# zju3dv/OnePose_Plus_Plus

Measured on NVIDIA H100. Metric: query images/sec (512x512, 5k 3D pts), higher is better.
Workload: dtype fp16 hi+lo operand pairs, 3 wgmma MMAs per K-step, fp32 accumulate (fp32-grade)

## Files before the change

### onepose_plus_plus_b200/csrc/opp_gemm.cu

```cuda
#include <cstdarg>
#include <cstdio>
#include <cstdlib>
#include <cstring>
#include <mutex>

#include "../../include/opp_b200.h"
#include "opp_gemm.cuh"

namespace opp {

static thread_local char g_last_error[512] = "";
void set_last_error(const char* fmt, ...) {
  va_list ap;
  va_start(ap, fmt);
  vsnprintf(g_last_error, sizeof(g_last_error), fmt, ap);
  va_end(ap);
}
const char* last_error() { return g_last_error; }

typedef CUresult (*EncodeTiledFn)(CUtensorMap*, CUtensorMapDataType, cuuint32_t, void*,
                                  const cuuint64_t*, const cuuint64_t*, const cuuint32_t*,
                                  const cuuint32_t*, CUtensorMapInterleave, CUtensorMapSwizzle,
                                  CUtensorMapL2promotion, CUtensorMapFloatOOBfill);

static EncodeTiledFn get_encode_fn() {
  static EncodeTiledFn fn = nullptr;
  static std::once_flag once;
  std::call_once(once, [] {
    void* p = nullptr;
    cudaDriverEntryPointQueryResult q;
    if (cudaGetDriverEntryPoint("cuTensorMapEncodeTiled", &p, cudaEnableDefault, &q) ==
            cudaSuccess &&
        q == cudaDriverEntryPointSuccess)
      fn = reinterpret_cast<EncodeTiledFn>(p);
  });
  return fn;
}

int num_sms() {
  static int n = 0;
  if (n == 0) {
    int dev = 0;
    if (cudaGetDevice(&dev) != cudaSuccess) return 132;
    if (cudaDeviceGetAttribute(&n, cudaDevAttrMultiProcessorCount, dev) != cudaSuccess) n = 132;
  }
  return n;
}

static int make_map(CUtensorMap* map, const void* ptr, int rank, const uint64_t* dims,
                    const uint64_t* strides_elems, const uint32_t* box) {
  EncodeTiledFn fn = get_encode_fn();
  if (!fn) {
    set_last_error("cuTensorMapEncodeTiled entry point unavailable (no CUDA driver?)");
    return OPP_ERR_CUDA;
  }
  OPP_REQUIRE((reinterpret_cast<uintptr_t>(ptr) & 15) == 0, "TMA base pointer not 16B aligned");
  OPP_REQUIRE(box[0] == 64 || box[0] == 32, "TMA inner box %u is not one swizzle row", box[0]);
  cuuint64_t gdim[5], gstr[4];
  cuuint32_t bdim[5], estr[5];
  for (int i = 0; i < rank; ++i) {
    gdim[i] = dims[i];
    bdim[i] = box[i];
    estr[i] = 1;
    OPP_REQUIRE(box[i] >= 1 && box[i] <= 256, "TMA box dim %d = %u out of range", i, box[i]);
  }
  for (int i = 0; i + 1 < rank; ++i) {
    gstr[i] = strides_elems[i] * 2;
    OPP_REQUIRE((gstr[i] & 15) == 0, "TMA stride %d (%llu B) not a multiple of 16", i,
                (unsigned long long)gstr[i]);
  }
  CUresult r = fn(map, CU_TENSOR_MAP_DATA_TYPE_FLOAT16, rank, const_cast<void*>(ptr), gdim, gstr,
                  bdim, estr, CU_TENSOR_MAP_INTERLEAVE_NONE,
                  box[0] == 32 ? CU_TENSOR_MAP_SWIZZLE_64B : CU_TENSOR_MAP_SWIZZLE_128B,
                  CU_TENSOR_MAP_L2_PROMOTION_L2_256B, CU_TENSOR_MAP_FLOAT_OOB_FILL_NONE);
  if (r != CUDA_SUCCESS) {
    set_last_error("cuTensorMapEncodeTiled failed with CUresult %d (rank %d dims %llu %llu %llu)",
                   (int)r, rank, (unsigned long long)dims[0], (unsigned long long)dims[1],
                   (unsigned long long)(rank > 2 ? dims[2] : 0));
    return OPP_ERR_CUDA;
  }
  return OPP_OK;
}

static int map_rows(CUtensorMap* map, const void* ptr, long long k, long long rows,
                    long long batches, long long ld, long long batch_stride, int box_rows, int bk = kBlockK) {
  uint64_t dims[3] = {(uint64_t)k, (uint64_t)rows, (uint64_t)batches};
  uint64_t str[2] = {(uint64_t)ld, (uint64_t)batch_stride};
  uint32_t box[3] = {(uint32_t)bk, (uint32_t)box_rows, 1};
  return make_map(map, ptr, 3, dims, str, box);
}

static void log_tile_once(int a_mode, const GemmShape& s, const char* epi) {
  static int on = -1;
  if (on < 0) {
    const char* e = getenv("OPP_LOG_TILES");
    on = e ? atoi(e) : 0;
  }
  if (!on) return;
  static std::mutex mu;
  static char seen[256][128];
  static int n_seen = 0;
  char key[128];
  snprintf(key, sizeof(key), "mode %d n %d block_n %d mma_n %d k %d conv_c %d stages %d alias %d cluster %d pair %d bk %d",
           a_mode, s.n_total, s.block_n, s.mma_n, s.k_chunks * kBlockK, s.conv_c, s.stages, s.acc_alias,
           s.cluster, s.pair, s.bk);
  std::lock_guard<std::mutex> lock(mu);
  if (on == 2) {
    fprintf(stderr, "opp gemm tile: %s epi %s\n", key, epi);
    return;
  }
  for (int i = 0; i < n_seen; ++i)
    if (!strcmp(seen[i], key)) return;
  if (n_seen < 256) strcpy(seen[n_seen++], key);
  fprintf(stderr, "opp gemm tile: %s\n", key);
}

template <int A_MODE, class Epi, bool DYN = false>
static int launch(const TensorMaps& maps, GemmShape s, const typename Epi::Params& ep,
                  cudaStream_t stream, const int* rows_dev = nullptr, int rows_mult = 1) {
  {
    static int dbg = -1;
    if (dbg < 0) {
      const char* e = getenv("OPP_DEBUG_SKIP");
      dbg = e ? atoi(e) : 0;
    }
    s.debug_skip = dbg;
    static int cap = -1;
    if (cap < 0) {
      const char* e = getenv("OPP_STAGES");
      cap = e ? atoi(e) : 0;
    }
    OPP_REQUIRE(s.mma_n >= EpiMinMmaN<Epi>::value, "GEMM tile width %d below the epilogue's minimum %d",
                s.mma_n, EpiMinMmaN<Epi>::value);
    OPP_REQUIRE(s.mma_n > 0 && gemm_pick_stages<Epi>(s, cap),
                "GEMM tile N=%d (split %d) does not fit in shared memory", s.block_n, s.split);
  }
  const int smem = gemm_smem_bytes<Epi>(s);
  log_tile_once(A_MODE, s, Epi::kName);
  OPP_REQUIRE(s.bk == kBlockK || (s.bk == 32 && A_MODE != A_ROWS), "ring slot width %d not compiled for mode %d",
              s.bk, A_MODE);
  const void* kern;
  if constexpr (DYN) kern = (const void*)gemm_kernel_dyn<A_MODE, Epi>;
  else kern = (const void*)gemm_kernel<A_MODE, Epi>;
  if constexpr (A_MODE != A_ROWS) {
    if (s.bk == 32) {
      if constexpr (DYN) kern = (const void*)gemm_kernel_dyn<A_MODE, Epi, 32>;
      else kern = (const void*)gemm_kernel<A_MODE, Epi, 32>;
    }
  }
  static unsigned long long attr_done[2] = {0, 0};
  unsigned long long& done = attr_done[s.bk == 32];
  int dev = 0;
  OPP_CHECK_CUDA(cudaGetDevice(&dev));
  if (dev < 64 && !((done >> dev) & 1ull)) {
    OPP_CHECK_CUDA(
        cudaFuncSetAttribute(kern, cudaFuncAttributeMaxDynamicSharedMemorySize, 227 * 1024));
    done |= 1ull << dev;
  }
  const long long total = (long long)s.batches * s.msup * s.n_tiles;
  if (total == 0) return OPP_OK;
  const int max_clusters = num_sms() / s.cluster;
  const int n_clusters = (int)(total < max_clusters ? total : max_clusters);
  cudaLaunchConfig_t cfg = {};
  cfg.gridDim = dim3(n_clusters * s.cluster);
  cfg.blockDim = dim3(gemm_threads(Epi::kGroups));
  cfg.dynamicSmemBytes = smem;
  cfg.stream = stream;
  cudaLaunchAttribute attr[2];
  attr[0].id = cudaLaunchAttributeClusterDimension;
  attr[0].val.clusterDim.x = s.cluster;
  attr[0].val.clusterDim.y = 1;
  attr[0].val.clusterDim.z = 1;
  attr[1].id = cudaLaunchAttributeProgrammaticStreamSerialization;
  attr[1].val.programmaticStreamSerializationAllowed = 1;
  cfg.attrs = attr;
  cfg.numAttrs = pdl_enabled() ? 2 : 1;
  void* kargs[5] = {(void*)&maps, (void*)&s, (void*)&ep, (void*)&rows_dev, (void*)&rows_mult};
  cudaError_t le = cudaLaunchKernelExC(&cfg, kern, kargs);
  if (le != cudaSuccess) {
    set_last_error("cudaLaunchKernelEx failed: %s (grid %d cluster %d pair %d smem %d stages %d "
                   "acc_alias %d block_n %d m_tiles %d n_tiles %d batches %d)",
                   cudaGetErrorString(le), n_clusters * s.cluster, s.cluster, s.pair, smem, s.stages,
                   s.acc_alias, s.block_n, s.m_tiles, s.n_tiles, s.batches);
    return OPP_ERR_CUDA;
  }
  return OPP_OK;
}

static int pick_cluster(int block_n, int m_tiles);

static void pick_grouping(GemmShape& s) {
  s.pair = 0;
  s.cluster = pick_cluster(s.block_n, s.m_tiles);
  s.msup = (s.m_tiles + s.cluster - 1) / s.cluster;
}

static int pick_cluster(int block_n, int m_tiles) {
  static int forced = -1;
  if (forced < 0) {
    const char* e = getenv("OPP_CLUSTER");
    forced = e ? atoi(e) : 0;
  }
  int c = forced > 1 ? forced : 2;
  while (c > 1 && (mma_width_for(block_n) % (8 * c) != 0 || m_tiles < c)) c >>= 1;
  return c;
}

static int conv_chunk_k(int ksize, int c_out_pad) {
  static int forced = -1;
  if (forced < 0) {
    const char* e = getenv("OPP_CONV_BK");
    forced = e ? atoi(e) : 0;
  }
  if (forced == 32 || forced == 64) return forced;
  return ksize == 3 && c_out_pad > 128 ? 32 : 64;
}

static int pick_block_n(int n) {
  if (n <= 256) return (n + 15) & ~15;
  if (n % 256 == 0) return 256;
  if (n % 128 == 0) return 128;
  return 256;
}

static void split_n_for_latency(GemmShape& s) {
  static int on = -1;
  if (on < 0) {
    const char* e = getenv("OPP_NSPLIT");
    on = e ? atoi(e) : 1;
  }
  if (!on) return;
  const int max_clusters = num_sms() / s.cluster;
  while (s.block_n >= 128 && s.block_n % 64 == 0 && s.n_total % (s.block_n / 2) == 0 &&
         (long long)s.batches * s.msup * s.n_tiles * 2 <= max_clusters) {
    s.block_n /= 2;
    s.n_tiles = s.n_total / s.block_n;
  }
}

static void ln_nsplit_cluster(GemmShape& s) {
  static int on = -1;
  if (on < 0) {
    const char* e = getenv("OPP_LN_NSPLIT");
    on = e ? atoi(e) : 1;
  }
  if (!on || s.n_total != 256 || s.block_n != 256) return;
  if ((long long)s.batches * s.m_tiles > num_sms() / 2) return;
  s.pair = 2;
  s.cluster = 2;
  s.msup = s.m_tiles;
  s.block_n = 128;
  s.n_tiles = 1;
}

template <class Epi>
static int fit_tile(GemmShape& s, int min_mma_n = 64) {
  for (;;) {
    s.mma_n = mma_width_for(s.block_n);
    if (s.mma_n < min_mma_n) s.mma_n = min_mma_n;
    GemmShape t = s;
    if (gemm_pick_stages<Epi>(t)) return OPP_OK;
    OPP_REQUIRE(s.pair == 0 && s.block_n > 16, "GEMM tile N=%d (split %d) does not fit in shared memory",
                s.block_n, s.split);
    s.block_n = (s.block_n / 2 + 15) & ~15;
    s.n_tiles = (s.n_total + s.block_n - 1) / s.block_n;
  }
}

static int setup_rows(TensorMaps& maps, GemmShape& s, const void* a0, int k0, const void* a1,
                      int k1, const void* w, int w_batched, int batches, long long rows, int n,
                      int split, int n_align = 16, int a0_shared = 0, int nsplit_ok = 0,
                      int min_mma_n = 64) {
  OPP_REQUIRE(a0 && w, "null operand");
  OPP_REQUIRE(k0 > 0 && k0 % 64 == 0 && k1 % 64 == 0, "K (%d,%d) must be multiples of 64", k0,
              k1);
  OPP_REQUIRE(n > 0 && n % n_align == 0, "N=%d must be a multiple of %d", n, n_align);
  OPP_REQUIRE(batches > 0 && rows > 0, "empty GEMM");
  const int planes = split ? 2 : 1;
  memset(&s, 0, sizeof(s));
  s.batches = batches;
  s.rows = (int)rows;
  s.m_tiles = (int)((rows + kBlockM - 1) / kBlockM);
  s.block_n = pick_block_n(n);
  OPP_REQUIRE(s.block_n % 16 == 0 && s.block_n <= 256, "bad block_n %d", s.block_n);
  s.n_tiles = (n + s.block_n - 1) / s.block_n;
  s.n_total = n;
  s.bk = kBlockK;
  s.k_chunks_a0 = k0 / 64;
  s.k_chunks = (k0 + k1) / 64;
  s.b_batched = w_batched;
  s.split = split ? 1 : 0;
  s.a0_lo = k0;
  s.a1_lo = k1;
  s.b_lo = k0 + k1;
  s.a0_shared = a0_shared ? 1 : 0;
  const long long ld0 = (long long)planes * k0, ld1 = (long long)planes * k1;
  int rc = map_rows(&maps.a[0], a0, ld0, rows, a0_shared ? 1 : batches, ld0, rows * ld0, kBlockM);
  if (rc) return rc;
  if (k1 > 0) {
    OPP_REQUIRE(a1, "null second A operand");
    rc = map_rows(&maps.a[1], a1, ld1, rows, batches, ld1, rows * ld1, kBlockM);
    if (rc) return rc;
  } else {
    maps.a[1] = maps.a[0];
  }
  maps.a[2] = maps.a[0];
  maps.a[3] = maps.a[0];
  pick_grouping(s);
  if (nsplit_ok == 1) split_n_for_latency(s);
  if (nsplit_ok == 2) ln_nsplit_cluster(s);
  rc = fit_tile<EpiLN>(s, min_mma_n);
  if (rc) return rc;
  const long long kt = (long long)planes * (k0 + k1);
  return map_rows(&maps.b, w, kt, n, w_batched ? batches : 1, kt, (long long)n * kt,
                  s.pair == 2 ? s.mma_n : s.mma_n / s.cluster);
}

}

using namespace opp;

extern "C" {

const char* opp_last_error(void) { return opp::last_error(); }

int opp_linear_act_f16(const void* a0, int k0, const void* a1, int k1, const void* w, void* out,
                       long long rows, int n, int act, int act_cols, int split,
                       opp_stream_t stream) {
  return opp_linear_act_f16_b(a0, k0, 0, a1, k1, w, out, 1, rows, n, act, act_cols, split, nullptr, stream);
}

int opp_linear_act_f16_b(const void* a0, int k0, int a0_shared, const void* a1, int k1, const void* w,
                         void* out, int batches, long long rows, int n, int act, int act_cols,
                         int split, const unsigned char* row_mask, opp_stream_t stream) {
  TensorMaps maps;
  GemmShape s;
  int rc = setup_rows(maps, s, a0, k0, a1, k1, w, 0, batches, rows, n, split, 16, a0_shared, 1);
  if (rc) return rc;
  OPP_REQUIRE(out, "null output");
  OPP_REQUIRE(act_cols % 32 == 0, "act_cols=%d must be a multiple of 32", act_cols);
  EpiStoreF16::Params ep{(__half*)out, (long long)n * (split ? 2 : 1), split ? n : 0, act,
                         act_cols, row_mask};
  return launch<A_ROWS, EpiStoreF16>(maps, s, ep, (cudaStream_t)stream);
}

int opp_linear_act_f16_out1(const void* a0, int k0, const void* a1, int k1, const void* w, void* out,
                            long long rows, int n, int act, int act_cols, const unsigned char* row_mask,
                            opp_stream_t stream) {
  TensorMaps maps;
  GemmShape s;
  int rc = setup_rows(maps, s, a0, k0, a1, k1, w, 0, 1, rows, n, 1, 16, 0, 1);
  if (rc) return rc;
  OPP_REQUIRE(out, "null output");
  OPP_REQUIRE(act_cols % 32 == 0, "act_cols=%d must be a multiple of 32", act_cols);
  EpiStoreF16::Params ep{(__half*)out, (long long)n, 0, act, act_cols, row_mask};
  return launch<A_ROWS, EpiStoreF16>(maps, s, ep, (cudaStream_t)stream);
}

int opp_linear_act_f16_dyn(const void* a0, int k0, const void* a1, int k1, const void* w, void* out,
                           long long cap_rows, const int* count, int rows_per_count, int n, int act,
                           int act_cols, int split, opp_stream_t stream) {
  TensorMaps maps;
  GemmShape s;
  int rc = setup_rows(maps, s, a0, k0, a1, k1, w, 0, 1, cap_rows, n, split);
  if (rc) return rc;
  OPP_REQUIRE(out && count && rows_per_count > 0, "bad dynamic-row arguments");
  OPP_REQUIRE(act_cols % 32 == 0, "act_cols=%d must be a multiple of 32", act_cols);
  EpiStoreF16::Params ep{(__half*)out, (long long)n * (split ? 2 : 1), split ? n : 0, act, act_cols, nullptr};
  return launch<A_ROWS, EpiStoreF16, true>(maps, s, ep, (cudaStream_t)stream, count, rows_per_count);
}

int opp_linear_ln_dyn(const void* a0, int k0, const void* a1, int k1, const void* w, const float* gamma,
                      const float* beta, float eps, const void* resid, void* out16, float* out32,
                      long long cap_rows, const int* count, int rows_per_count, int n, int split,
                      opp_stream_t stream) {
  TensorMaps maps;
  GemmShape s;
  OPP_REQUIRE(n == 128 || n == 256, "LayerNorm epilogue needs N in {128,256}, got %d", n);
  int rc = setup_rows(maps, s, a0, k0, a1, k1, w, 0, 1, cap_rows, n, split);
  if (rc) return rc;
  OPP_REQUIRE(s.n_tiles == 1 && s.block_n == n, "LayerNorm row of N=%d split across tiles", n);
  OPP_REQUIRE(gamma && beta && count && rows_per_count > 0, "bad dynamic-row arguments");
  OPP_REQUIRE(out16 || out32, "no output requested");
  EpiLN::Params ep{gamma, beta, eps, (const __half*)resid, 0, (__half*)out16,
                   (long long)n * (split ? 2 : 1), split ? n : 0, out32};
  return launch<A_ROWS, EpiLN, true>(maps, s, ep, (cudaStream_t)stream, count, rows_per_count);
}

int opp_linear_q_f16(const void* x, const void* wq, const float* ksum, void* out, int batches,
                     int rows, int d_model, float v_len, float eps, int split, int x_shared,
                     const unsigned char* row_mask, opp_stream_t stream) {
  TensorMaps maps;
  GemmShape s;
  OPP_REQUIRE(d_model == 256, "opp_linear_q_f16 supports d_model 256 (8 heads x 32), got %d",
              d_model);
  int rc = setup_rows(maps, s, x, d_model, nullptr, 0, wq, 0, batches, rows, d_model, split, 16, x_shared, 1);
  if (rc) return rc;
  OPP_REQUIRE(ksum && out, "null pointer");
  EpiQ::Params ep{(__half*)out, (long long)d_model * (split ? 2 : 1), split ? d_model : 0, ksum,
                  v_len, eps, row_mask};
  return launch<A_ROWS, EpiQ>(maps, s, ep, (cudaStream_t)stream);
}

int opp_linear_ln(const void* a0, int k0, const void* a1, int k1, const void* w, int w_batched,
                  const float* gamma, const float* beta, float eps, const void* resid,
                  int resid_shared, void* out16, float* out32, int batches, long long rows, int n,
                  int split, opp_stream_t stream) {
  TensorMaps maps;
  GemmShape s;
  OPP_REQUIRE(n == 128 || n == 256, "LayerNorm epilogue needs N in {128,256}, got %d", n);
  int rc = setup_rows(maps, s, a0, k0, a1, k1, w, w_batched, batches, rows, n, split, 16, 0, 2);
  if (rc) return rc;
  OPP_REQUIRE(s.n_tiles == 1 && s.block_n * (s.pair == 2 ? 2 : 1) == n,
              "LayerNorm row of N=%d split across tiles", n);
  OPP_REQUIRE(gamma && beta, "null LayerNorm parameters");
  OPP_REQUIRE(out16 || out32, "no output requested");
  EpiLN::Params ep{gamma, beta, eps, (const __half*)resid, resid_shared, (__half*)out16,
                   (long long)n * (split ? 2 : 1), split ? n : 0, out32};
  return launch<A_ROWS, EpiLN>(maps, s, ep, (cudaStream_t)stream);
}

int opp_conv2d_nhwc(const void* in, const void* w, const float* bias, const void* resid,
                    void* out, int batch, int in_h, int in_w, int c_in_pad, int c_out_pad,
                    int ksize, int stride, int act, float slope, void* tok, const float* pe,
                    const void* up, int split, opp_stream_t stream) {
  OPP_REQUIRE(in && w && bias, "null operand");
  OPP_REQUIRE(ksize == 1 || ksize == 3, "kernel size %d unsupported (1 or 3)", ksize);
  OPP_REQUIRE(stride == 1 || stride == 2, "stride %d unsupported", stride);
  OPP_REQUIRE(c_in_pad % 16 == 0 && c_out_pad % 16 == 0 && c_out_pad <= 256,
              "channel counts must be padded to multiples of 16 (got %d -> %d)", c_in_pad,
              c_out_pad);
  OPP_REQUIRE(stride == 1 || (in_h % 2 == 0 && in_w % 2 == 0), "stride 2 needs even H, W");
  OPP_REQUIRE(out || tok, "no output requested");
  const int planes = split ? 2 : 1;
  const int pad = ksize / 2;
  const int out_h = (in_h + 2 * pad - ksize) / stride + 1;
  const int out_w = (in_w + 2 * pad - ksize) / stride + 1;
  TensorMaps maps;
  GemmShape s;
  memset(&s, 0, sizeof(s));
  s.batches = batch;
  s.rows = out_h * out_w;
  s.tile_w = 16;
  s.tile_h = 8;
  s.tiles_x = (out_w + s.tile_w - 1) / s.tile_w;
  s.tiles_y = (out_h + s.tile_h - 1) / s.tile_h;
  s.m_tiles = s.tiles_x * s.tiles_y;
  s.block_n = c_out_pad;
  s.n_tiles = 1;
  s.n_total = c_out_pad;
  s.conv_c = c_in_pad;
  s.bk = conv_chunk_k(ksize, c_out_pad);
  s.conv_cchunks = (c_in_pad + 63) / 64;
  s.k_chunks = ksize * ksize * s.conv_cchunks;
  s.conv_kw = ksize;
  s.conv_pad = pad;
  s.conv_stride = stride;
  s.out_w = out_w;
  s.out_h = out_h;
  s.split = split ? 1 : 0;
  const long long C = (long long)planes * c_in_pad;
  const __half* base = (const __half*)in;
  int rc;
  if (stride == 1) {
    uint64_t dims[5] = {(uint64_t)c_in_pad, (uint64_t)planes, (uint64_t)in_w, (uint64_t)in_h, (uint64_t)batch};
    uint64_t str[4] = {(uint64_t)c_in_pad, (uint64_t)C, (uint64_t)(in_w * C), (uint64_t)((long long)in_h * in_w * C)};
    uint32_t box[5] = {(uint32_t)s.bk, 1, (uint32_t)s.tile_w, (uint32_t)s.tile_h, 1};
    rc = make_map(&maps.a[0], base, 5, dims, str, box);
    if (rc) return rc;
    maps.a[1] = maps.a[2] = maps.a[3] = maps.a[0];
  } else {
    for (int py = 0; py < 2; ++py)
      for (int px = 0; px < 2; ++px) {
        uint64_t dims[5] = {(uint64_t)c_in_pad, (uint64_t)planes, (uint64_t)(in_w / 2),
                            (uint64_t)(in_h / 2), (uint64_t)batch};
        uint64_t str[4] = {(uint64_t)c_in_pad, (uint64_t)(2 * C), (uint64_t)(2LL * in_w * C),
                           (uint64_t)((long long)in_h * in_w * C)};
        uint32_t box[5] = {(uint32_t)s.bk, 1, (uint32_t)s.tile_w, (uint32_t)s.tile_h, 1};
        rc = make_map(&maps.a[py * 2 + px], base + ((long long)py * in_w + px) * C, 5, dims, str,
                      box);
        if (rc) return rc;
      }
  }
  const long long kplane = (long long)ksize * ksize * c_in_pad;
  s.b_lo = (int)kplane;
  const long long kt = kplane * planes;
  pick_grouping(s);
  split_n_for_latency(s);
  rc = up ? fit_tile<EpiConvUp>(s) : fit_tile<EpiConv>(s);
  if (rc) return rc;
  rc = map_rows(&maps.b, w, kt, c_out_pad, 1, kt, (long long)c_out_pad * kt, s.mma_n / s.cluster, s.bk);
  if (rc) return rc;
  OPP_REQUIRE(!up || (out_h % 2 == 0 && out_w % 2 == 0 && out_h >= 4 && out_w >= 4),
              "fused upsample-add needs even output dims >= 4 (got %d x %d)", out_h, out_w);
  EpiConvParams ep{(__half*)out, (long long)c_out_pad * planes, split ? c_out_pad : 0, bias,
                     (const __half*)resid, act, slope, (__half*)tok, pe, (const __half*)up,
                     out_h / 2, out_w / 2,
                     up ? (float)(out_h / 2 - 1) / (float)(out_h - 1) : 0.f,
                     up ? (float)(out_w / 2 - 1) / (float)(out_w - 1) : 0.f};
  if (up) return launch<A_CONV, EpiConvUp>(maps, s, ep, (cudaStream_t)stream);
  return launch<A_CONV, EpiConv>(maps, s, ep, (cudaStream_t)stream);
}

int opp_conv_win_pitch(int win) {
  static int pack5 = -1;
  if (pack5 < 0) {
    const char* e = getenv("OPP_WIN5_PACK");
    pack5 = e ? atoi(e) : 0;
  }
  return (win == 5 && pack5) ? 5 : 8;
}

int opp_conv_win(const void* in, const void* w, const float* bias, void* out, const long long* b_ids,
                 const long long* j_ids, int matches, const int* count, int batch, int in_h, int in_w,
                 int c_in_pad, int c_out_pad, int win, int wc, int stride, int org, int act,
                 float slope, int split, opp_stream_t stream) {
  OPP_REQUIRE(in && w && bias && out, "null operand");
  OPP_REQUIRE(win == 5 || win == 7, "window side %d unsupported (5 or 7)", win);
  OPP_REQUIRE(c_in_pad % 16 == 0 && c_out_pad % 16 == 0 && c_out_pad <= 256,
              "channel counts must be padded to multiples of 16 (got %d -> %d)", c_in_pad, c_out_pad);
  OPP_REQUIRE(matches >= 0 && (j_ids == nullptr) == (b_ids == nullptr), "bad match list");
  OPP_REQUIRE(!j_ids || (wc > 0 && stride > 0 && batch > 0 && in_h > 0 && in_w > 0),
              "dense-input window convolution needs the map size, wc and stride");
  if (matches == 0) return OPP_OK;
  const int planes = split ? 2 : 1;
  TensorMaps maps;
  GemmShape s;
  memset(&s, 0, sizeof(s));
  s.batches = 1;
  const int pitch = opp_conv_win_pitch(win);
  s.tile_w = pitch;
  s.tile_h = win;
  s.tiles_x = 128 / (pitch * win);
  s.tiles_y = 1;
  s.rows = matches * pitch * win;
  s.m_tiles = (matches + s.tiles_x - 1) / s.tiles_x;
  s.block_n = c_out_pad;
  s.n_tiles = 1;
  s.n_total = c_out_pad;
  s.conv_c = c_in_pad;
  s.bk = conv_chunk_k(3, c_out_pad);
  OPP_REQUIRE(pitch == 8 || s.bk == 64, "OPP_WIN5_PACK needs 64-wide ring slots (layer has %d)", s.bk);
  s.conv_cchunks = (c_in_pad + 63) / 64;
  s.k_chunks = 9 * s.conv_cchunks;
  s.conv_kw = 3;
  s.conv_pad = 1;
  s.conv_stride = 1;
  s.out_w = pitch;
  s.out_h = win;
  s.split = split ? 1 : 0;
  const long long C = (long long)planes * c_in_pad;
  int rc;
  {
    const uint64_t iw = j_ids ? in_w : 8, ih = j_ids ? in_h : win + 2, ib = j_ids ? batch : matches;
    uint64_t dims[5] = {(uint64_t)c_in_pad, (uint64_t)planes, iw, ih, ib};
    uint64_t str[4] = {(uint64_t)c_in_pad, (uint64_t)C, (uint64_t)(iw * C), (uint64_t)(ih * iw * C)};
    uint32_t box[5] = {(uint32_t)s.bk, 1, (uint32_t)pitch, (uint32_t)win, 1};
    rc = make_map(&maps.a[0], in, 5, dims, str, box);
    if (rc) return rc;
    maps.a[1] = maps.a[2] = maps.a[3] = maps.a[0];
  }
  const long long kplane = 9LL * c_in_pad;
  s.b_lo = (int)kplane;
  const long long kt = kplane * planes;
  pick_grouping(s);
  rc = fit_tile<EpiWin>(s);
  if (rc) return rc;
  rc = map_rows(&maps.b, w, kt, c_out_pad, 1, kt, (long long)c_out_pad * kt, s.mma_n / s.cluster, s.bk);
  if (rc) return rc;
  EpiWin::Params ep{(__half*)out, (long long)c_out_pad * planes, split ? c_out_pad : 0, bias, act, slope,
                    b_ids, j_ids, wc, stride, org, in_h, in_w};
  if (count) return launch<A_WIN, EpiWin, true>(maps, s, ep, (cudaStream_t)stream, count, pitch * win);
  return launch<A_WIN, EpiWin>(maps, s, ep, (cudaStream_t)stream);
}

int opp_sim_lse(const void* a, const void* b, float* part_m, float* part_s, int batches, int rows,
                int cols, int k, float scale, int split, opp_stream_t stream) {
  TensorMaps maps;
  GemmShape s;
  int rc = setup_rows(maps, s, a, k, nullptr, 0, b, 1, batches, rows, cols, split, 1);
  if (rc) return rc;
  EpiLse::Params ep{part_m, part_s, scale};
  return launch<A_ROWS, EpiLse>(maps, s, ep, (cudaStream_t)stream);
}

int opp_sim_conf(const void* a, const void* b, const float* lse_own, const float* lse_other,
                 int own_is_pt, float* conf, float* part_val, int* part_idx, int batches,
                 int rows, int cols, int k, float scale, int split, opp_stream_t stream) {
  TensorMaps maps;
  GemmShape s;
  int rc = setup_rows(maps, s, a, k, nullptr, 0, b, 1, batches, rows, cols, split, 1);
  if (rc) return rc;
  EpiConf::Params ep{lse_own, lse_other, scale, own_is_pt, conf, part_val, part_idx};
  return launch<A_ROWS, EpiConf>(maps, s, ep, (cudaStream_t)stream);
}

int opp_sim_lse_cols_rows(const void* a, const void* b, float* part_m, float* part_s, float* col_m,
                          float* col_s, int batches, int rows, int cols, int k, float scale, int split,
                          const unsigned char* col_mask, const int* row_count, opp_stream_t stream) {
  TensorMaps maps;
  GemmShape s;
  int rc = setup_rows(maps, s, a, k, nullptr, 0, b, 1, batches, rows, cols, split, 1, 0, 0,
                      EpiLseCol::kMinMmaN);
  if (rc) return rc;
  OPP_REQUIRE(part_m && part_s && col_m && col_s, "null pointer");
  OPP_REQUIRE(!(col_mask && row_count), "col_mask and row_count are not combined");
  EpiLseColParams ep{part_m, part_s, scale, col_m, col_s, (rows + 31) / 32, col_mask};
  if (row_count) {
    EpiLseColRowsParams epr{ep, row_count};
    return launch<A_ROWS, EpiLseColRows>(maps, s, epr, (cudaStream_t)stream);
  }
  if (col_mask) return launch<A_ROWS, EpiLseColMasked>(maps, s, ep, (cudaStream_t)stream);
  return launch<A_ROWS, EpiLseCol>(maps, s, ep, (cudaStream_t)stream);
}

int opp_sim_lse_cols(const void* a, const void* b, float* part_m, float* part_s, float* col_m,
                     float* col_s, int batches, int rows, int cols, int k, float scale, int split,
                     const unsigned char* col_mask, opp_stream_t stream) {
  return opp_sim_lse_cols_rows(a, b, part_m, part_s, col_m, col_s, batches, rows, cols, k, scale, split,
                               col_mask, nullptr, stream);
}

int opp_sim_conf_colmax_rows(const void* a, const void* b, const float* lse_own, const float* lse_other,
                             float* conf, float* part_val, int* part_idx, unsigned* colmax, int batches,
                             int rows, int cols, int k, float scale, int split, const int* row_count,
                             opp_stream_t stream) {
  TensorMaps maps;
  GemmShape s;
  int rc = setup_rows(maps, s, a, k, nullptr, 0, b, 1, batches, rows, cols, split, 1, 0, 0,
                      EpiConfCol::kMinMmaN);
  if (rc) return rc;
  OPP_REQUIRE(lse_own && lse_other && part_val && part_idx && colmax, "null pointer");
  OPP_CHECK_CUDA(cudaMemsetAsync(colmax, 0, (size_t)batches * cols * sizeof(unsigned),
                                 (cudaStream_t)stream));
  EpiConfColParams ep{lse_own, lse_other, scale, conf, part_val, part_idx, colmax};
  if (row_count) {
    EpiConfColRowsParams epr{ep, row_count};
    return launch<A_ROWS, EpiConfColRows>(maps, s, epr, (cudaStream_t)stream);
  }
  return launch<A_ROWS, EpiConfCol>(maps, s, ep, (cudaStream_t)stream);
}

int opp_sim_conf_colmax(const void* a, const void* b, const float* lse_own, const float* lse_other,
                        float* conf, float* part_val, int* part_idx, unsigned* colmax, int batches,
                        int rows, int cols, int k, float scale, int split, opp_stream_t stream) {
  return opp_sim_conf_colmax_rows(a, b, lse_own, lse_other, conf, part_val, part_idx, colmax, batches, rows,
                                  cols, k, scale, split, nullptr, stream);
}

int opp_sim_tiles(int cols) {
  return (cols + pick_block_n(cols) - 1) / pick_block_n(cols);
}

}
```

### onepose_plus_plus_b200/csrc/opp_gemm.cuh

```cuda
#pragma once

#include <type_traits>

#include "opp_common.cuh"

#ifndef OPP_CONV_GROUPS
#define OPP_CONV_GROUPS 2
#endif

namespace opp {

constexpr int kBlockM = 128;
constexpr int kBlockK = 64;
__host__ __device__ constexpr int gemm_a_bytes(int bk) { return kBlockM * bk * 2; }
constexpr int kMaxStages = 8;
constexpr int kEpiParamBytes = 4096;
constexpr int kMaxEpiWarps = 8;
constexpr int gemm_threads(int groups) { return 128 + 128 * groups; }
constexpr int kProducerRegs = 40;
constexpr int kMmaRegs = 232;
static_assert(128 * kProducerRegs + 256 * kMmaRegs <= 65536, "register file of one SM");
constexpr int kMmaWidths[] = {64, 128, 208, 256};
constexpr int mma_width_for(int block_n) {
  for (int w : kMmaWidths)
    if (w >= block_n) return w;
  return 0;
}

enum AMode : int { A_ROWS = 0, A_CONV = 1, A_WIN = 2 };

struct TensorMaps {
  CUtensorMap a[4];
  CUtensorMap b;
};

struct GemmShape {
  int batches;
  int rows;
  int m_tiles;
  int n_tiles;
  int n_total;
  int block_n;
  int mma_n;
  int k_chunks;
  int bk;
  int stages;
  int b_batched;
  int cluster;
  int msup;
  int pair;
  int acc_alias;
  int debug_skip;
  int split;
  int b_lo;
  int k_chunks_a0;
  int a0_lo, a1_lo;
  int a0_shared;
  int conv_cchunks;
  int conv_c;
  int conv_kw;
  int conv_pad;
  int conv_stride;
  int tile_w, tile_h;
  int tiles_x, tiles_y;
  int out_w, out_h;
};

struct EpiCtx {
  uint32_t acc;
  int b, m_tile, n_tile;
  int q;
  int a_mode;
  int n0;
  int ncols;
  int etid;
  float* smem;
  uint8_t* wstage;
  uint32_t smem_s, wstage_s;
  int group;
  int col_first, col_step;
  long long sgrow[4];
  unsigned svalid;
  int next_b, next_m_tile;
  uint8_t* extra;
  int it;
};

__device__ __forceinline__ void epi_sync(const EpiCtx& c) { named_bar_sync(1 + c.group, 128); }

template <class E, class = void>
struct EpiWarpStage {
  static constexpr int value = 32 * 80;
};
template <class E>
struct EpiWarpStage<E, std::void_t<decltype(E::kWarpStage)>> {
  static constexpr int value = E::kWarpStage;
};
template <class E, class = void>
struct EpiExtraSmem {
  static constexpr int value = 0;
};
template <class E>
struct EpiExtraSmem<E, std::void_t<decltype(E::kExtraSmem)>> {
  static constexpr int value = E::kExtraSmem;
};
template <class E>
constexpr int epi_smem_bytes() {
  return 4096 + 8 * EpiWarpStage<E>::value + EpiExtraSmem<E>::value;
}

template <class E, class = void>
struct EpiMinMmaN {
  static constexpr int value = 64;
};
template <class E>
struct EpiMinMmaN<E, std::void_t<decltype(E::kMinMmaN)>> {
  static constexpr int value = E::kMinMmaN;
};

template <class E, class = void>
struct EpiNeedsNext : std::false_type {};
template <class E>
struct EpiNeedsNext<E, std::void_t<decltype(E::kNeedsNext)>> : std::true_type {};

template <class E, class = void>
struct EpiFromRegs : std::false_type {};
template <class E>
struct EpiFromRegs<E, std::void_t<decltype(E::kFromRegs)>> : std::true_type {};

__device__ __forceinline__ bool epi_row_at(const GemmShape& s, const EpiCtx& c, int rit,
                                           long long& grow, int& row) {
  bool ok;
  if (c.a_mode == A_ROWS) {
    row = c.m_tile * kBlockM + rit;
    ok = row < s.rows;
  } else if (c.a_mode == A_WIN) {
    const int wrows = s.tiles_x * s.tile_w * s.tile_h;
    row = c.m_tile * wrows + rit;
    ok = rit < wrows && row < s.rows;
  } else {
    const int ty = c.m_tile / s.tiles_x;
    const int tx = c.m_tile - ty * s.tiles_x;
    const int ly = rit / s.tile_w;
    const int oy = ty * s.tile_h + ly;
    const int ox = tx * s.tile_w + (rit - ly * s.tile_w);
    ok = oy < s.out_h && ox < s.out_w;
    row = oy * s.out_w + ox;
  }
  grow = (long long)c.b * s.rows + row;
  return ok;
}

constexpr int kAccPad = 4;
__host__ __device__ constexpr int gemm_acc_bytes(int mma_n) { return 128 * (mma_n + kAccPad) * 4; }

__device__ __forceinline__ void acc_ld32(uint32_t waddr, float (&v)[32]) {
#pragma unroll
  for (int i = 0; i < 8; ++i) {
    const uint4 u = lds128(waddr * 4 + 16 * i);
    v[4 * i + 0] = __uint_as_float(u.x);
    v[4 * i + 1] = __uint_as_float(u.y);
    v[4 * i + 2] = __uint_as_float(u.z);
    v[4 * i + 3] = __uint_as_float(u.w);
  }
}

constexpr int kStageRowH = 80;
constexpr int kWarpStageBytes = 32 * kStageRowH;

__device__ __forceinline__ void staged_store_h32(const GemmShape& s, const EpiCtx& c, __half* out,
                                                 long long ld, int lo_off, int gcol,
                                                 const float* v, int nvalid) {
  if (s.debug_skip & 8) return;
  const int lane = threadIdx.x & 31;
  const uint32_t st = c.wstage_s;
#pragma unroll
  for (int plane = 0; plane < 2; ++plane) {
    if (plane == 1 && lo_off == 0) break;
    const uint32_t mine = st + lane * kStageRowH;
#pragma unroll
    for (int g = 0; g < 4; ++g) {
      uint4 u;
      if (plane == 0) {
        u.x = pack_half2(v[8 * g + 0], v[8 * g + 1]);
        u.y = pack_half2(v[8 * g + 2], v[8 * g + 3]);
        u.z = pack_half2(v[8 * g + 4], v[8 * g + 5]);
        u.w = pack_half2(v[8 * g + 6], v[8 * g + 7]);
      } else {
        float l[8];
#pragma unroll
        for (int j = 0; j < 8; ++j)
          l[j] = v[8 * g + j] - __half2float(__float2half_rn(v[8 * g + j]));
        u.x = pack_half2(l[0], l[1]);
        u.y = pack_half2(l[2], l[3]);
        u.z = pack_half2(l[4], l[5]);
        u.w = pack_half2(l[6], l[7]);
      }
      sts128(mine + g * 16, u);
    }
    __syncwarp();
    const int seg = lane & 3;
#pragma unroll
    for (int i = 0; i < 4; ++i) {
      const int rr = (lane >> 2) + 8 * i;
      if (((c.svalid >> i) & 1u) && seg * 8 < nvalid)
        *reinterpret_cast<uint4*>(out + c.sgrow[i] * ld + plane * lo_off + gcol + seg * 8) =
            lds128(st + rr * kStageRowH + seg * 16);
    }
    __syncwarp();
  }
}


constexpr int kFragRowH = 80;
constexpr int kFragPlaneH = 16 * kFragRowH;
constexpr int kFragRowF = 160;

__device__ __forceinline__ void sts32u(uint32_t addr, uint32_t v) {
  asm volatile("st.shared.b32 [%0], %1;" ::"r"(addr), "r"(v) : "memory");
}
__device__ __forceinline__ uint32_t lds32u(uint32_t addr) {
  uint32_t v;
  asm volatile("ld.shared.b32 %0, [%1];" : "=r"(v) : "r"(addr) : "memory");
  return v;
}
__device__ __forceinline__ float2 lds64f(uint32_t addr) {
  float2 v;
  asm volatile("ld.shared.v2.f32 {%0, %1}, [%2];" : "=f"(v.x), "=f"(v.y) : "r"(addr) : "memory");
  return v;
}

__device__ __forceinline__ void sts64f(uint32_t addr, float a, float b) {
  asm volatile("st.shared.v2.f32 [%0], {%1, %2};" ::"r"(addr), "f"(a), "f"(b) : "memory");
}

template <int N>
__device__ __forceinline__ void frag_slice(const float (&d)[N / 2], int j, float (&v)[16], float fill = 0.f) {
#pragma unroll
  for (int k = 0; k < 16; ++k) v[k] = 16 * j + k < N / 2 ? d[16 * j + k] : fill;
}

__device__ __forceinline__ void frag_add_cols(uint32_t base_s, int col, float (&v)[16]) {
  const int c0 = 2 * (threadIdx.x & 3);
#pragma unroll
  for (int ii = 0; ii < 4; ++ii) {
    const float2 b = lds64f(base_s + 4 * ((col + 8 * ii + c0) & 255));
#pragma unroll
    for (int h = 0; h < 2; ++h) {
      v[4 * ii + 2 * h] += b.x;
      v[4 * ii + 2 * h + 1] += b.y;
    }
  }
}

__device__ __forceinline__ void frag_store_h(const GemmShape& s, const EpiCtx& c, __half* out, long long ld,
                                             int lo_off, int gcol, const float (&v)[16], int nvalid) {
  if (s.debug_skip & 8) return;
  const int lane = threadIdx.x & 31, t = lane & 3, rq = lane >> 2;
  const uint32_t st = c.wstage_s;
#pragma unroll
  for (int ii = 0; ii < 4; ++ii)
#pragma unroll
    for (int h = 0; h < 2; ++h) {
      const float a = v[4 * ii + 2 * h], b = v[4 * ii + 2 * h + 1];
      const uint32_t addr = st + (rq + 8 * h) * kFragRowH + 16 * ii + 4 * t;
      sts32u(addr, pack_half2(a, b));
      if (lo_off)
        sts32u(addr + kFragPlaneH, pack_half2(a - __half2float(__float2half_rn(a)),
                                              b - __half2float(__float2half_rn(b))));
    }
  __syncwarp();
#pragma unroll
  for (int plane = 0; plane < 2; ++plane) {
    if (plane == 1 && lo_off == 0) break;
#pragma unroll
    for (int h = 0; h < 2; ++h)
      if (((c.svalid >> h) & 1u) && t * 8 < nvalid)
        *reinterpret_cast<uint4*>(out + c.sgrow[h] * ld + plane * lo_off + gcol + t * 8) =
            lds128(st + plane * kFragPlaneH + (rq + 8 * h) * kFragRowH + 16 * t);
  }
  __syncwarp();
}

__device__ __forceinline__ void frag_store_f32(const EpiCtx& c, float* out, long long ld, int gcol,
                                               const float (&v)[16], int nvalid) {
  const int lane = threadIdx.x & 31, t = lane & 3, rq = lane >> 2;
  const uint32_t st = c.wstage_s;
#pragma unroll
  for (int ii = 0; ii < 4; ++ii)
#pragma unroll
    for (int h = 0; h < 2; ++h)
      sts64f(st + (rq + 8 * h) * kFragRowF + 4 * (8 * ii + 2 * t), v[4 * ii + 2 * h], v[4 * ii + 2 * h + 1]);
  __syncwarp();
#pragma unroll
  for (int half = 0; half < 2; ++half)
#pragma unroll
    for (int h = 0; h < 2; ++h)
      if (((c.svalid >> h) & 1u) && 16 * half + 4 * t < nvalid)
        *reinterpret_cast<uint4*>(out + c.sgrow[h] * ld + gcol + 16 * half + 4 * t) =
            lds128(st + (rq + 8 * h) * kFragRowF + 64 * half + 16 * t);
  __syncwarp();
}

__device__ __forceinline__ void frag_load_issue(const EpiCtx& c, const __half* src, long long ld, int lo_off,
                                                int gcol, int nvalid) {
  const int lane = threadIdx.x & 31, t = lane & 3, rq = lane >> 2;
#pragma unroll
  for (int h = 0; h < 2; ++h) {
    const bool in = ((c.svalid >> h) & 1u) && t * 8 < nvalid;
    const __half* row = in ? src + c.sgrow[h] * ld + gcol + t * 8 : src;
    const uint32_t dst = c.wstage_s + (rq + 8 * h) * kFragRowH + 16 * t;
    cp_async16_zfill(dst, row, in ? 16 : 0);
    if (lo_off) cp_async16_zfill(dst + kFragPlaneH, in ? row + lo_off : src, in ? 16 : 0);
  }
  cp_async_commit();
}
__device__ __forceinline__ void frag_load_add(const EpiCtx& c, int lo_off, float (&v)[16]) {
  const int lane = threadIdx.x & 31, t = lane & 3, rq = lane >> 2;
  const uint32_t st = c.wstage_s;
  cp_async_wait<0>();
  __syncwarp();
#pragma unroll
  for (int plane = 0; plane < 2; ++plane) {
    if (plane == 1 && lo_off == 0) break;
#pragma unroll
    for (int ii = 0; ii < 4; ++ii)
#pragma unroll
      for (int h = 0; h < 2; ++h) {
        const uint32_t u = lds32u(st + plane * kFragPlaneH + (rq + 8 * h) * kFragRowH + 16 * ii + 4 * t);
        const float2 f = __half22float2(*reinterpret_cast<const __half2*>(&u));
        v[4 * ii + 2 * h] += f.x;
        v[4 * ii + 2 * h + 1] += f.y;
      }
  }
  __syncwarp();
}

__device__ __forceinline__ void frag_add_f32(const EpiCtx& c, const float* src, long long ld, const int (&row)[2],
                                             int gcol, int nvalid, float (&v)[16]) {
  const int lane = threadIdx.x & 31, t = lane & 3, rq = lane >> 2;
  const uint32_t st = c.wstage_s;
#pragma unroll
  for (int h = 0; h < 2; ++h)
#pragma unroll
    for (int k = 0; k < 2; ++k) {
      const int seg = t + 4 * k;
      if (((c.svalid >> h) & 1u) && seg * 4 < nvalid)
        sts128(st + (rq + 8 * h) * kFragRowF + 16 * seg,
               *reinterpret_cast<const uint4*>(src + (long long)row[h] * ld + gcol + seg * 4));
    }
  __syncwarp();
#pragma unroll
  for (int h = 0; h < 2; ++h) {
    if (!((c.svalid >> h) & 1u)) continue;
#pragma unroll
    for (int ii = 0; ii < 4; ++ii)
      if (8 * ii < nvalid) {
        const float2 f = lds64f(st + (rq + 8 * h) * kFragRowF + 4 * (8 * ii + 2 * t));
        v[4 * ii + 2 * h] += f.x;
        v[4 * ii + 2 * h + 1] += f.y;
      }
  }
  __syncwarp();
}

__device__ __forceinline__ void frag_act(int act, float slope, float (&v)[16]) {
  if (act == 1) {
#pragma unroll
    for (int k = 0; k < 16; ++k) v[k] = fmaxf(v[k], 0.f);
  } else if (act == 2) {
#pragma unroll
    for (int k = 0; k < 16; ++k) v[k] = v[k] > 0.f ? v[k] : v[k] * slope;
  }
}

__device__ __forceinline__ void epi_stage_cols(const GemmShape& s, const EpiCtx& c, const float* src) {
  if (c.it > 0 && s.n_tiles == 1) return;
  epi_sync(c);
  for (int i = c.etid; i < c.ncols; i += 128) sts32f(c.smem_s + 4 * i, src[c.n0 + i]);
  epi_sync(c);
}

struct EpiConvParams {
  __half* out;
  long long ld;
  int out_lo;
  const float* bias;
  const __half* resid;
  int act;
  float slope;
  __half* tok;
  const float* pe;
  const __half* up;
  int up_h, up_w;
  float up_sy, up_sx;
};
struct EpiConv {
  static constexpr int kGroups = OPP_CONV_GROUPS;
  static constexpr const char* kName = "conv";
  static constexpr bool kFromRegs = true;
  using Params = EpiConvParams;
  __device__ static void prefetch(const Params& p, const GemmShape& s, const EpiCtx& c) {
    if (!p.resid) return;
    const int t = threadIdx.x & 3;
#pragma unroll
    for (int h = 0; h < 2; ++h) {
      if (!((c.svalid >> h) & 1u)) continue;
      const char* row = reinterpret_cast<const char*>(p.resid + c.sgrow[h] * p.ld + c.n0);
      for (int o = 128 * t; o < c.ncols * 2; o += 512) {
        asm volatile("prefetch.global.L2 [%0];" ::"l"(row + o));
        if (p.out_lo) asm volatile("prefetch.global.L2 [%0];" ::"l"(row + 2 * p.out_lo + o));
      }
    }
  }
  template <int N>
  __device__ __forceinline__ static void run_frag(const Params& p, const GemmShape& s, const EpiCtx& c, float (&d)[N / 2]) {
    const bool has_res = p.resid != nullptr;
    if (has_res) frag_load_issue(c, p.resid, p.ld, p.out_lo, c.n0, c.ncols);
    epi_stage_cols(s, c, p.bias);
    int prow[2] = {0, 0};
#pragma unroll
    for (int h = 0; h < 2; ++h) prow[h] = (int)(c.sgrow[h] - (long long)c.b * s.rows);
#pragma unroll
    for (int j = 0; j < (N + 31) / 32; ++j) {
      const int col = 32 * j;
      if (col < c.ncols) {
        const int g0 = c.n0 + col;
        const int nvalid = c.ncols - col;
        float v[16];
        frag_slice<N>(d, j, v);
        frag_add_cols(c.smem_s, col, v);
        if (has_res) frag_load_add(c, p.out_lo, v);
        frag_act(p.act, p.slope, v);
        if (p.out) frag_store_h(s, c, p.out, p.ld, p.out_lo, g0, v, nvalid);
        if (p.tok) {
          frag_add_f32(c, p.pe, s.n_total, prow, g0, nvalid, v);
          frag_store_h(s, c, p.tok, p.ld, p.out_lo, g0, v, nvalid);
        }
        if (has_res && col + 32 < c.ncols) frag_load_issue(c, p.resid, p.ld, p.out_lo, g0 + 32, nvalid - 32);
      }
    }
  }
};

struct EpiWin {
  static constexpr int kGroups = OPP_CONV_GROUPS;
  static constexpr const char* kName = "conv_win";
  static constexpr bool kFromRegs = true;
  struct Params {
    __half* out;
    long long ld;
    int out_lo;
    const float* bias;
    int act;
    float slope;
    const long long* b_ids;
    const long long* j_ids;
    int wc;
    int stride;
    int org;
    int in_h, in_w;
  };
  __device__ static void prefetch(const Params&, const GemmShape&, const EpiCtx&) {}
  template <int N>
  __device__ __forceinline__ static void run_frag(const Params& p, const GemmShape& s, const EpiCtx& c, float (&d)[N / 2]) {
    epi_stage_cols(s, c, p.bias);
    bool inside[2] = {true, true};
#pragma unroll
    for (int h = 0; h < 2; ++h) {
      if (p.j_ids && ((c.svalid >> h) & 1u)) {
        const int rpm = s.tile_w * s.tile_h;
        const int m = (int)(c.sgrow[h] / rpm);
        const int local = (int)(c.sgrow[h] - (long long)m * rpm);
        const int ly = local / s.tile_w, lx = local - ly * s.tile_w;
        const int jj = (int)p.j_ids[m];
        const int cy = jj / p.wc;
        const int y = p.stride * cy + p.org + ly, x = p.stride * (jj - cy * p.wc) + p.org + lx;
        inside[h] = y >= 0 && y < p.in_h && x >= 0 && x < p.in_w;
      }
    }
#pragma unroll
    for (int j = 0; j < (N + 31) / 32; ++j) {
      const int col = 32 * j;
      if (col < c.ncols) {
        float v[16];
        frag_slice<N>(d, j, v);
        frag_add_cols(c.smem_s, col, v);
        frag_act(p.act, p.slope, v);
#pragma unroll
        for (int h = 0; h < 2; ++h)
          if (!inside[h]) {
#pragma unroll
            for (int ii = 0; ii < 4; ++ii) v[4 * ii + 2 * h] = v[4 * ii + 2 * h + 1] = 0.f;
          }
        frag_store_h(s, c, p.out, p.ld, p.out_lo, c.n0 + col, v, c.ncols - col);
      }
    }
  }
};

struct EpiConvUp {
  static constexpr int kGroups = OPP_CONV_GROUPS;
  static constexpr const char* kName = "conv_up";
  static constexpr bool kNeedsNext = true;
  static constexpr int kWarpStage = 2 * 32 * 80;
  using Params = EpiConvParams;

  struct Geo {
    int ymin, xmin;
  };
  __device__ static Geo window(const Params& p, const GemmShape& s, int m_tile, int q) {
    const int ty = m_tile / s.tiles_x;
    const int oy = min(ty * s.tile_h + (q * 32) / s.tile_w, s.out_h - 1);
    const int ox = min((m_tile - ty * s.tiles_x) * s.tile_w, s.out_w - 1);
    return Geo{(int)(p.up_sy * (float)oy), (int)(p.up_sx * (float)ox)};
  }
  __device__ static long long slot_pixel(const Params& p, int b, const Geo& g, int slot) {
    const int sy_ = slot / 10, sx_ = slot - sy_ * 10;
    return ((long long)b * p.up_h + min(g.ymin + sy_, p.up_h - 1)) * p.up_w + min(g.xmin + sx_, p.up_w - 1);
  }
  __device__ static void prefetch(const Params& p, const GemmShape& s, const EpiCtx& c) {
    if (c.next_b < 0) return;
    const int lane = threadIdx.x & 31;
    if (lane >= 30) return;
    const Geo g = window(p, s, c.next_m_tile, c.q);
    const char* px = reinterpret_cast<const char*>(p.up + slot_pixel(p, c.next_b, g, lane) * p.ld);
    const int bytes = (p.out_lo ? 2 : 1) * s.n_total * 2;
    for (int o = c.group * 128; o < bytes; o += 128 * kGroups) asm volatile("prefetch.global.L2 [%0];" ::"l"(px + o));
  }
  __device__ static void run(const Params& p, const GemmShape& s, const EpiCtx& c) {
    epi_sync(c);
    for (int i = c.etid; i < c.ncols; i += 128) sts32f(c.smem_s + 4 * i, p.bias[c.n0 + i]);
    epi_sync(c);
    const int lane = threadIdx.x & 31;
    const int seg = lane & 3;
    const Geo g = window(p, s, c.m_tile, c.q);
    float w00, w01, w10, w11;
    uint32_t a00, a01, a10, a11;
    {
      const int rit = c.q * 32 + lane;
      const int ty = c.m_tile / s.tiles_x;
      const int ly = rit / s.tile_w;
      const int oy = min(ty * s.tile_h + ly, s.out_h - 1);
      const int ox = min((c.m_tile - ty * s.tiles_x) * s.tile_w + (rit - ly * s.tile_w), s.out_w - 1);
      const float fy = p.up_sy * (float)oy, fx = p.up_sx * (float)ox;
      const int y0 = (int)fy, x0 = (int)fx;
      const int y1 = y0 + (y0 < p.up_h - 1 ? 1 : 0), x1 = x0 + (x0 < p.up_w - 1 ? 1 : 0);
      const float wy = fy - (float)y0, wx = fx - (float)x0;
      w00 = (1.f - wy) * (1.f - wx);
      w01 = (1.f - wy) * wx;
      w10 = wy * (1.f - wx);
      w11 = wy * wx;
      a00 = c.wstage_s + ((y0 - g.ymin) * 10 + (x0 - g.xmin)) * kStageRowH;
      a01 = c.wstage_s + ((y0 - g.ymin) * 10 + (x1 - g.xmin)) * kStageRowH;
      a10 = c.wstage_s + ((y1 - g.ymin) * 10 + (x0 - g.xmin)) * kStageRowH;
      a11 = c.wstage_s + ((y1 - g.ymin) * 10 + (x1 - g.xmin)) * kStageRowH;
    }
    int spix[4];
#pragma unroll
    for (int i = 0; i < 4; ++i) spix[i] = (int)slot_pixel(p, c.b, g, min((lane >> 2) + 8 * i, 29));
    const __half* upb = p.up + seg * 8 + c.n0;
    const bool two = p.out_lo != 0;
    uint4 nb[8];
    auto issue = [&](int col) {
      const bool ok = seg * 8 < c.ncols - col;
#pragma unroll
      for (int i = 0; i < 4; ++i) {
        const __half* px = upb + (long long)spix[i] * p.ld + col;
        nb[i] = ok ? *reinterpret_cast<const uint4*>(px) : make_uint4(0, 0, 0, 0);
        nb[4 + i] = (ok && two) ? *reinterpret_cast<const uint4*>(px + p.out_lo) : make_uint4(0, 0, 0, 0);
      }
    };
    constexpr uint32_t kLo = 32 * kStageRowH;
    auto stage = [&]() {
#pragma unroll
      for (int i = 0; i < 4; ++i) {
        const uint32_t a = c.wstage_s + ((lane >> 2) + 8 * i) * kStageRowH + seg * 16;
        sts128(a, nb[i]);
        if (two) sts128(a + kLo, nb[4 + i]);
      }
      __syncwarp();
    };
    auto blend = [&](float* v) {
#pragma unroll
      for (int q4 = 0; q4 < 4; ++q4) {
#pragma unroll
        for (int plane = 0; plane < 2; ++plane) {
          if (plane == 1 && !two) break;
          const uint32_t o = plane * kLo + q4 * 16;
          const uint4 q00 = lds128(a00 + o), q01 = lds128(a01 + o);
          const uint4 q10 = lds128(a10 + o), q11 = lds128(a11 + o);
          const __half2* h00 = reinterpret_cast<const __half2*>(&q00);
          const __half2* h01 = reinterpret_cast<const __half2*>(&q01);
          const __half2* h10 = reinterpret_cast<const __half2*>(&q10);
          const __half2* h11 = reinterpret_cast<const __half2*>(&q11);
#pragma unroll
          for (int j = 0; j < 4; ++j) {
            const float2 fa = __half22float2(h00[j]), fb = __half22float2(h01[j]);
            const float2 fc = __half22float2(h10[j]), fd = __half22float2(h11[j]);
            v[8 * q4 + 2 * j] += (w00 * fa.x + w01 * fb.x) + (w10 * fc.x + w11 * fd.x);
            v[8 * q4 + 2 * j + 1] += (w00 * fa.y + w01 * fb.y) + (w10 * fc.y + w11 * fd.y);
          }
        }
      }
      __syncwarp();
    };
    if (c.col_first < c.ncols) issue(c.col_first);
    for (int col = c.col_first; col < c.ncols; col += c.col_step) {
      float v[32];
      acc_ld32(c.acc + col, v);
#pragma unroll
      for (int q4 = 0; q4 < 8; ++q4) {
        const uint4 bq = lds128(c.smem_s + 4 * ((col + 4 * q4) & 255));
        v[4 * q4 + 0] += __uint_as_float(bq.x);
        v[4 * q4 + 1] += __uint_as_float(bq.y);
        v[4 * q4 + 2] += __uint_as_float(bq.z);
        v[4 * q4 + 3] += __uint_as_float(bq.w);
      }
      stage();
      const int ncol = col + c.col_step;
      if (ncol < c.ncols) issue(ncol);
      blend(v);
      if (p.act == 1) {
#pragma unroll
        for (int j = 0; j < 32; ++j) v[j] = fmaxf(v[j], 0.f);
      } else if (p.act == 2) {
#pragma unroll
        for (int j = 0; j < 32; ++j) v[j] = v[j] > 0.f ? v[j] : v[j] * p.slope;
      }
      staged_store_h32(s, c, p.out, p.ld, p.out_lo, c.n0 + col, v, c.ncols - col);
    }
  }
};

__device__ __forceinline__ float quad_sum(float x) {
  x += __shfl_xor_sync(0xffffffffu, x, 1);
  return x + __shfl_xor_sync(0xffffffffu, x, 2);
}
__device__ __forceinline__ float quad_max(float x) {
  x = fmaxf(x, __shfl_xor_sync(0xffffffffu, x, 1));
  return fmaxf(x, __shfl_xor_sync(0xffffffffu, x, 2));
}
__device__ __forceinline__ void quad_argmax(float& v, int& idx) {
#pragma unroll
  for (int o = 1; o <= 2; o <<= 1) {
    const float ov = __shfl_xor_sync(0xffffffffu, v, o);
    const int oi = __shfl_xor_sync(0xffffffffu, idx, o);
    if (ov > v || (ov == v && oi < idx)) {
      v = ov;
      idx = oi;
    }
  }
}

template <class Op>
__device__ __forceinline__ void col_allreduce8(float (&x)[8], Op op) {
#pragma unroll
  for (int o = 4; o <= 16; o <<= 1)
#pragma unroll
    for (int k = 0; k < 8; ++k) x[k] = op(x[k], __shfl_xor_sync(0xffffffffu, x[k], o));
}
template <class Op>
__device__ __forceinline__ float col_reduce8(float (&x)[8], Op op) {
  const int lane = threadIdx.x & 31;
#pragma unroll
  for (int lvl = 2; lvl >= 0; --lvl) {
    const int half = 1 << lvl;
    const bool up = (lane >> (2 + lvl)) & 1;
#pragma unroll
    for (int k = 0; k < half; ++k) {
      const float keep = up ? x[half + k] : x[k];
      const float send = up ? x[k] : x[half + k];
      x[k] = op(keep, __shfl_xor_sync(0xffffffffu, send, 4 << lvl));
    }
  }
  return x[0];
}
__device__ __forceinline__ int frag_lane_col() {
  const int lane = threadIdx.x & 31, rq = lane >> 2;
  return 8 * (rq >> 1) + 2 * (lane & 3) + (rq & 1);
}
__device__ __forceinline__ float pick8(const float (&x)[8], int k) {
  float r = x[0];
#pragma unroll
  for (int i = 1; i < 8; ++i) r = k == i ? x[i] : r;
  return r;
}
__device__ __forceinline__ void pair_sync(const EpiCtx& c) { named_bar_sync(5 + 2 * c.group + (c.q >> 1), 64); }

__device__ __forceinline__ void epi_stage_cols_b(const GemmShape& s, const EpiCtx& c, const float* src) {
  epi_sync(c);
  for (int i = c.etid; i < c.ncols; i += 128) sts32f(c.smem_s + 4 * i, src[(long long)c.b * s.n_total + c.n0 + i]);
  epi_sync(c);
}

struct EpiStoreF16 {
  static constexpr int kGroups = 2;
  static constexpr const char* kName = "store_f16";
  static constexpr bool kFromRegs = true;
  struct Params {
    __half* out;
    long long ld;
    int out_lo;
    int act;
    int act_cols;
    const unsigned char* row_mask;
  };
  __device__ static void prefetch(const Params&, const GemmShape&, const EpiCtx&) {}
  template <int N>
  __device__ __forceinline__ static void run_frag(const Params& p, const GemmShape& s, const EpiCtx& c, float (&d)[N / 2]) {
    bool masked[2] = {false, false};
#pragma unroll
    for (int h = 0; h < 2; ++h) masked[h] = p.row_mask && ((c.svalid >> h) & 1u) && p.row_mask[c.sgrow[h]] == 0;
#pragma unroll
    for (int j = 0; j < (N + 31) / 32; ++j) {
      const int col = 32 * j;
      if (col < c.ncols) {
        const int g0 = c.n0 + col;
        const int act = g0 < p.act_cols ? p.act : 0;
        float v[16];
        frag_slice<N>(d, j, v);
        if (act == 1) {
#pragma unroll
          for (int k = 0; k < 16; ++k) v[k] = fmaxf(v[k], 0.f);
        } else if (act == 2) {
#pragma unroll
          for (int k = 0; k < 16; ++k) v[k] = elu_plus_one_fast(v[k]);
        }
#pragma unroll
        for (int h = 0; h < 2; ++h)
          if (masked[h]) {
#pragma unroll
            for (int ii = 0; ii < 4; ++ii) v[4 * ii + 2 * h] = v[4 * ii + 2 * h + 1] = 0.f;
          }
        frag_store_h(s, c, p.out, p.ld, p.out_lo, g0, v, c.ncols - col);
      }
    }
  }
};

struct EpiQ {
  static constexpr int kGroups = 2;
  static constexpr const char* kName = "q";
  static constexpr bool kFromRegs = true;
  struct Params {
    __half* out;
    long long ld;
    int out_lo;
    const float* ksum;
    float v_len;
    float eps;
    const unsigned char* row_mask;
  };
  __device__ static void prefetch(const Params&, const GemmShape&, const EpiCtx&) {}
  template <int N>
  __device__ __forceinline__ static void run_frag(const Params& p, const GemmShape& s, const EpiCtx& c, float (&d)[N / 2]) {
    epi_stage_cols_b(s, c, p.ksum);
    const int c0 = 2 * (threadIdx.x & 3);
    bool qmasked[2] = {false, false};
#pragma unroll
    for (int h = 0; h < 2; ++h) qmasked[h] = p.row_mask && ((c.svalid >> h) & 1u) && p.row_mask[c.sgrow[h]] == 0;
#pragma unroll
    for (int j = 0; j < (N + 31) / 32; ++j) {
      const int col = 32 * j;
      if (col < c.ncols) {
        float v[16];
        frag_slice<N>(d, j, v);
        float dot[2] = {0.f, 0.f};
#pragma unroll
        for (int ii = 0; ii < 4; ++ii) {
          const float2 kk = lds64f(c.smem_s + 4 * (col + 8 * ii + c0));
#pragma unroll
          for (int h = 0; h < 2; ++h) {
            v[4 * ii + 2 * h] = elu_plus_one_fast(v[4 * ii + 2 * h]);
            v[4 * ii + 2 * h + 1] = elu_plus_one_fast(v[4 * ii + 2 * h + 1]);
            dot[h] = fmaf(v[4 * ii + 2 * h], kk.x, dot[h]);
            dot[h] = fmaf(v[4 * ii + 2 * h + 1], kk.y, dot[h]);
          }
        }
#pragma unroll
        for (int h = 0; h < 2; ++h) {
          const float qd = quad_sum(dot[h]);
          const float z = qmasked[h] ? 0.f : p.v_len / (qd + p.eps);
#pragma unroll
          for (int ii = 0; ii < 4; ++ii) {
            v[4 * ii + 2 * h] *= z;
            v[4 * ii + 2 * h + 1] *= z;
          }
        }
        frag_store_h(s, c, p.out, p.ld, p.out_lo, c.n0 + col, v, 32);
      }
    }
  }
};

struct EpiLN {
  static constexpr int kGroups = 2;
  static constexpr const char* kName = "ln";
  static constexpr bool kFromRegs = true;
  static constexpr int kExtraSmem = 2 * 128 * 8 + 64;
  static constexpr int kExchangeArrivals = 64;
  struct Params {
    const float* gamma;
    const float* beta;
    float eps;
    const __half* resid;
    int resid_shared;
    __half* out16;
    long long ld;
    int out_lo;
    float* out32;
  };
  __device__ static void prefetch(const Params& p, const GemmShape& s, const EpiCtx& c) {
    if (!p.resid) return;
    const int t = threadIdx.x & 3;
#pragma unroll
    for (int h = 0; h < 2; ++h) {
      if (!((c.svalid >> h) & 1u)) continue;
      const long long r = p.resid_shared ? c.sgrow[h] - (long long)c.b * s.rows : c.sgrow[h];
      const char* row = reinterpret_cast<const char*>(p.resid + r * p.ld + c.n0);
      for (int o = 128 * t; o < c.ncols * 2; o += 512) {
        asm volatile("prefetch.global.L2 [%0];" ::"l"(row + o));
        if (p.out_lo) asm volatile("prefetch.global.L2 [%0];" ::"l"(row + 2 * p.out_lo + o));
      }
    }
  }
  template <int N>
  __device__ __forceinline__ static void run_frag(const Params& p, const GemmShape& s, const EpiCtx& c, float (&d)[N / 2]) {
    const int lane = threadIdx.x & 31, c0 = 2 * (lane & 3);
    const __half* resid = p.resid;
    if (resid && p.resid_shared) resid -= (long long)c.b * s.rows * p.ld;
    if (resid) frag_load_issue(c, resid, p.ld, p.out_lo, c.n0, c.ncols);
    if (c.it == 0) {
      for (int i = c.etid; i < c.ncols; i += 128) {
        sts32f(c.smem_s + 4 * i, p.gamma[c.n0 + i]);
        sts32f(c.smem_s + 4 * (256 + i), p.beta[c.n0 + i]);
      }
      epi_sync(c);
    }
    float mean[2], m2[2];
#pragma unroll
    for (int h = 0; h < 2; ++h) {
      float s1 = 0.f;
#pragma unroll
      for (int i = 0; i < N / 8; ++i) s1 += d[4 * i + 2 * h] + d[4 * i + 2 * h + 1];
      mean[h] = quad_sum(s1) / (float)c.ncols;
      float s2 = 0.f;
#pragma unroll
      for (int i = 0; i < N / 8; ++i) {
        const float a = d[4 * i + 2 * h] - mean[h], b = d[4 * i + 2 * h + 1] - mean[h];
        s2 = fmaf(a, a, s2);
        s2 = fmaf(b, b, s2);
      }
      m2[h] = quad_sum(s2);
    }
    if (s.pair == 2) {
      const int par = c.it & 1;
      const int r0 = 64 * c.group + 16 * c.q + (lane >> 2);
      float2* slot = reinterpret_cast<float2*>(c.extra) + par * 128 + r0;
      uint64_t* xbar = reinterpret_cast<uint64_t*>(c.extra + 2 * 128 * 8) + par;
      const uint32_t peer = (uint32_t)(c.n_tile ^ 1);
      float2 o[2] = {make_float2(0.f, 0.f), make_float2(0.f, 0.f)};
      if ((lane & 3) == 0) {
        st_cluster_f32x2(slot, peer, mean[0], m2[0]);
        st_cluster_f32x2(slot + 8, peer, mean[1], m2[1]);
        mbar_arrive_cluster_release(xbar, peer);
        mbar_wait_cluster(xbar, (uint32_t)((c.it >> 1) & 1));
        o[0] = slot[0];
        o[1] = slot[8];
      }
#pragma unroll
      for (int h = 0; h < 2; ++h) {
        o[h].x = __shfl_sync(0xffffffffu, o[h].x, lane & ~3);
        o[h].y = __shfl_sync(0xffffffffu, o[h].y, lane & ~3);
        const float mean_a = c.n_tile == 0 ? mean[h] : o[h].x, m2a = c.n_tile == 0 ? m2[h] : o[h].y;
        const float mean_b = c.n_tile == 0 ? o[h].x : mean[h], m2b = c.n_tile == 0 ? o[h].y : m2[h];
        const float delta = mean_b - mean_a;
        mean[h] = mean_a + delta * 0.5f;
        m2[h] = m2a + m2b + delta * delta * (0.5f * (float)c.ncols);
      }
    }
    float rstd[2];
#pragma unroll
    for (int h = 0; h < 2; ++h) rstd[h] = 1.f / sqrtf(m2[h] / (float)s.n_total + p.eps);
#pragma unroll
    for (int j = 0; j < (N + 31) / 32; ++j) {
      const int col = 32 * j;
      if (col < c.ncols) {
        const int nvalid = c.ncols - col;
        float v[16];
        frag_slice<N>(d, j, v);
#pragma unroll
        for (int ii = 0; ii < 4; ++ii) {
          const float2 gq = lds64f(c.smem_s + 4 * (col + 8 * ii + c0));
          const float2 bq = lds64f(c.smem_s + 4 * (256 + col + 8 * ii + c0));
#pragma unroll
          for (int h = 0; h < 2; ++h) {
            v[4 * ii + 2 * h] = (v[4 * ii + 2 * h] - mean[h]) * rstd[h] * gq.x + bq.x;
            v[4 * ii + 2 * h + 1] = (v[4 * ii + 2 * h + 1] - mean[h]) * rstd[h] * gq.y + bq.y;
          }
        }
        if (resid) frag_load_add(c, p.out_lo, v);
        if (p.out32) frag_store_f32(c, p.out32, s.n_total, c.n0 + col, v, nvalid);
        if (p.out16) frag_store_h(s, c, p.out16, p.ld, p.out_lo, c.n0 + col, v, nvalid);
        if (resid && col + 32 < c.ncols) frag_load_issue(c, resid, p.ld, p.out_lo, c.n0 + col + 32, nvalid - 32);
      }
    }
  }
};

struct EpiLse {
  static constexpr int kGroups = 2;
  static constexpr const char* kName = "lse";
  static constexpr bool kFromRegs = true;
  struct Params {
    float* part_m;
    float* part_s;
    float scale;
  };
  __device__ static void prefetch(const Params&, const GemmShape&, const EpiCtx&) {}
  template <int N>
  __device__ __forceinline__ static void run_frag(const Params& p, const GemmShape& s, const EpiCtx& c, float (&d)[N / 2]) {
    const int c0 = 2 * (threadIdx.x & 3);
#pragma unroll
    for (int h = 0; h < 2; ++h) {
      float m = -INFINITY;
#pragma unroll
      for (int i = 0; i < N / 8; ++i)
#pragma unroll
        for (int e = 0; e < 2; ++e)
          if (8 * i + c0 + e < c.ncols) m = fmaxf(m, d[4 * i + 2 * h + e] * p.scale);
      m = quad_max(m);
      float sum = 0.f;
#pragma unroll
      for (int i = 0; i < N / 8; ++i)
#pragma unroll
        for (int e = 0; e < 2; ++e)
          if (8 * i + c0 + e < c.ncols) sum += fast_exp(d[4 * i + 2 * h + e] * p.scale - m);
      sum = quad_sum(sum);
      if ((threadIdx.x & 3) == 0 && ((c.svalid >> h) & 1u)) {
        p.part_m[c.sgrow[h] * s.n_tiles + c.n_tile] = m;
        p.part_s[c.sgrow[h] * s.n_tiles + c.n_tile] = sum;
      }
    }
  }
};

__device__ __forceinline__ void conf_store(const GemmShape& s, const EpiCtx& c, float* conf, int col,
                                           const float (&v)[16]) {
  if ((s.n_total & 3) == 0) {
    frag_store_f32(c, conf, (long long)s.n_total, c.n0 + col, v, c.ncols - col);
    return;
  }
  const int c0 = 2 * (threadIdx.x & 3);
#pragma unroll
  for (int h = 0; h < 2; ++h) {
    if (!((c.svalid >> h) & 1u)) continue;
    float* dst = conf + c.sgrow[h] * (long long)s.n_total + c.n0 + col;
#pragma unroll
    for (int ii = 0; ii < 4; ++ii)
#pragma unroll
      for (int e = 0; e < 2; ++e)
        if (col + 8 * ii + c0 + e < c.ncols) dst[8 * ii + c0 + e] = v[4 * ii + 2 * h + e];
  }
}

__device__ __forceinline__ void conf_slice(const EpiCtx& c, int col, float scale, const float (&lown)[2],
                                           bool own_is_pt, float (&v)[16], float (&best)[2], int (&bidx)[2]) {
  const int c0 = 2 * (threadIdx.x & 3);
#pragma unroll
  for (int ii = 0; ii < 4; ++ii)
#pragma unroll
    for (int e = 0; e < 2; ++e) {
      const int cl = col + 8 * ii + c0 + e;
      const float lo = lds32f(c.smem_s + 4 * (cl & 255));
#pragma unroll
      for (int h = 0; h < 2; ++h) {
        const float x2 = 2.f * (v[4 * ii + 2 * h + e] * scale);
        const float x = fast_exp(own_is_pt ? (x2 - lown[h]) - lo : (x2 - lo) - lown[h]);
        v[4 * ii + 2 * h + e] = x;
        if (cl < c.ncols && x > best[h]) {
          best[h] = x;
          bidx[h] = c.n0 + cl;
        }
      }
    }
}
__device__ __forceinline__ void conf_best_store(const GemmShape& s, const EpiCtx& c, float* part_val, int* part_idx,
                                                float (&best)[2], int (&bidx)[2]) {
#pragma unroll
  for (int h = 0; h < 2; ++h) {
    quad_argmax(best[h], bidx[h]);
    if ((threadIdx.x & 3) == 0 && ((c.svalid >> h) & 1u)) {
      part_val[c.sgrow[h] * s.n_tiles + c.n_tile] = best[h];
      part_idx[c.sgrow[h] * s.n_tiles + c.n_tile] = bidx[h];
    }
  }
}

struct EpiConf {
  static constexpr int kGroups = 2;
  static constexpr const char* kName = "conf";
  static constexpr bool kFromRegs = true;
  struct Params {
    const float* lse_own;
    const float* lse_other;
    float scale;
    int own_is_pt;
    float* conf;
    float* part_val;
    int* part_idx;
  };
  __device__ static void prefetch(const Params&, const GemmShape&, const EpiCtx&) {}
  template <int N>
  __device__ __forceinline__ static void run_frag(const Params& p, const GemmShape& s, const EpiCtx& c, float (&d)[N / 2]) {
    epi_stage_cols_b(s, c, p.lse_other);
    float lown[2], best[2] = {-1.f, -1.f};
    int bidx[2] = {c.n0, c.n0};
#pragma unroll
    for (int h = 0; h < 2; ++h) lown[h] = ((c.svalid >> h) & 1u) ? p.lse_own[c.sgrow[h]] : 0.f;
#pragma unroll
    for (int j = 0; j < (N + 31) / 32; ++j) {
      const int col = 32 * j;
      if (col < c.ncols) {
        float v[16];
        frag_slice<N>(d, j, v);
        conf_slice(c, col, p.scale, lown, p.own_is_pt != 0, v, best, bidx);
        if (p.conf) conf_store(s, c, p.conf, col, v);
      }
    }
    conf_best_store(s, c, p.part_val, p.part_idx, best, bidx);
  }
};

struct EpiLseColParams {
  float* part_m;
  float* part_s;
  float scale;
  float* col_m;
  float* col_s;
  int row_groups;
  const unsigned char* col_mask;
};
struct EpiLseColRowsParams : EpiLseColParams {
  const int* row_count;
};

__device__ __forceinline__ unsigned rows_below_count(const GemmShape& s, const EpiCtx& c, const int* row_count) {
  const long long end = (long long)c.b * s.rows + row_count[c.b];
  return c.svalid & ((c.sgrow[0] < end ? 1u : 0u) | (c.sgrow[1] < end ? 2u : 0u));
}

template <bool kMask, bool kRows = false>
struct EpiLseColT {
  static_assert(!(kMask && kRows), "query_image_mask and per-batch row counts are not combined");
  static constexpr int kGroups = 2;
  static constexpr const char* kName = kRows ? "lse_col_rows" : "lse_col";
  static constexpr bool kFromRegs = true;
  static constexpr int kMinMmaN = 128;
  using Params = std::conditional_t<kRows, EpiLseColRowsParams, EpiLseColParams>;
  __device__ static void prefetch(const Params&, const GemmShape&, const EpiCtx&) {}
  template <int N>
  __device__ __forceinline__ static void run_frag(const Params& p, const GemmShape& s, const EpiCtx& c, float (&d)[N / 2]) {
    const int lane = threadIdx.x & 31, c0 = 2 * (lane & 3);
    unsigned valid = c.svalid;
    if constexpr (kRows) valid = rows_below_count(s, c, p.row_count);
    if constexpr (kMask) {
      epi_sync(c);
      for (int i = c.etid; i < c.ncols; i += 128)
        sts32f(c.smem_s + 4 * i, p.col_mask[(long long)c.b * s.n_total + c.n0 + i] ? 0.f : -1e9f);
      epi_sync(c);
    }
#pragma unroll
    for (int i = 0; i < N / 8; ++i)
#pragma unroll
      for (int e = 0; e < 2; ++e) {
        const int cl = 8 * i + c0 + e;
        float cb_ = 0.f;
        if constexpr (kMask) cb_ = lds32f(c.smem_s + 4 * (cl & 255));
#pragma unroll
        for (int h = 0; h < 2; ++h)
          d[4 * i + 2 * h + e] = (((valid >> h) & 1u) && cl < c.ncols) ? d[4 * i + 2 * h + e] * p.scale + cb_
                                                                        : -INFINITY;
      }
#pragma unroll
    for (int h = 0; h < 2; ++h) {
      float m = -INFINITY;
#pragma unroll
      for (int i = 0; i < N / 8; ++i) m = fmaxf(m, fmaxf(d[4 * i + 2 * h], d[4 * i + 2 * h + 1]));
      m = quad_max(m);
      float sum = 0.f;
#pragma unroll
      for (int i = 0; i < N / 8; ++i)
#pragma unroll
        for (int e = 0; e < 2; ++e)
          if (8 * i + c0 + e < c.ncols) sum += fast_exp(d[4 * i + 2 * h + e] - m);
      sum = quad_sum(sum);
      if ((lane & 3) == 0 && ((valid >> h) & 1u)) {
        p.part_m[c.sgrow[h] * s.n_tiles + c.n_tile] = m;
        p.part_s[c.sgrow[h] * s.n_tiles + c.n_tile] = sum;
      }
    }
    constexpr int kSlices = (N + 31) / 32;
    float cmax[kSlices], csum[kSlices];
    const int rq = lane >> 2;
#pragma unroll
    for (int j = 0; j < kSlices; ++j) {
      cmax[j] = -INFINITY;
      csum[j] = 0.f;
      if (32 * j < c.ncols) {
        float v[16];
        frag_slice<N>(d, j, v, -INFINITY);
        float x[8];
#pragma unroll
        for (int k = 0; k < 8; ++k) x[k] = fmaxf(v[4 * (k >> 1) + (k & 1)], v[4 * (k >> 1) + 2 + (k & 1)]);
        col_allreduce8(x, [](float a, float b) { return fmaxf(a, b); });
        cmax[j] = pick8(x, rq);
#pragma unroll
        for (int k = 0; k < 8; ++k) {
          const float a = v[4 * (k >> 1) + (k & 1)], b = v[4 * (k >> 1) + 2 + (k & 1)];
          x[k] = (a == -INFINITY ? 0.f : fast_exp(a - x[k])) + (b == -INFINITY ? 0.f : fast_exp(b - x[k]));
        }
        csum[j] = col_reduce8(x, [](float a, float b) { return a + b; });
      }
    }
    const bool odd = (c.q & 1) != 0;
    const uint32_t xs = c.wstage_s + (odd ? 0 : kWarpStageBytes);
    if (odd) {
#pragma unroll
      for (int j = 0; j < kSlices; ++j) sts64f(xs + 8 * (32 * j + lane), cmax[j], csum[j]);
    }
    pair_sync(c);
    if (!odd) {
      const int rg = c.m_tile * 4 + 2 * c.group + (c.q >> 1);
      if (rg < p.row_groups) {
        const long long cbase = ((long long)c.b * p.row_groups + rg) * s.n_total + c.n0;
        const int lc = frag_lane_col();
#pragma unroll
        for (int j = 0; j < kSlices; ++j) {
          const int cl = 32 * j + lc;
          if (cl < c.ncols) {
            const float2 o = lds64f(xs + 8 * (32 * j + lane));
            const float m = fmaxf(cmax[j], o.x);
            const float sa = cmax[j] == -INFINITY ? 0.f : csum[j] * fast_exp(cmax[j] - m);
            const float sb = o.x == -INFINITY ? 0.f : o.y * fast_exp(o.x - m);
            p.col_m[cbase + cl] = m;
            p.col_s[cbase + cl] = sa + sb;
          }
        }
      }
    }
    pair_sync(c);
  }
};

using EpiLseCol = EpiLseColT<false>;
using EpiLseColMasked = EpiLseColT<true>;
using EpiLseColRows = EpiLseColT<false, true>;

struct EpiConfColParams {
  const float* lse_own;
  const float* lse_other;
  float scale;
  float* conf;
  float* part_val;
  int* part_idx;
  unsigned* colmax;
};
struct EpiConfColRowsParams : EpiConfColParams {
  const int* row_count;
};
template <bool kRows>
struct EpiConfColT {
  static constexpr int kGroups = 2;
  static constexpr const char* kName = kRows ? "conf_col_rows" : "conf_col";
  static constexpr bool kFromRegs = true;
  static constexpr int kMinMmaN = 128;
  using Params = std::conditional_t<kRows, EpiConfColRowsParams, EpiConfColParams>;
  __device__ static void prefetch(const Params&, const GemmShape&, const EpiCtx&) {}
  template <int N>
  __device__ __forceinline__ static void run_frag(const Params& p, const GemmShape& s, const EpiCtx& c, float (&d)[N / 2]) {
    const int lane = threadIdx.x & 31;
    epi_stage_cols_b(s, c, p.lse_other);
    unsigned valid = c.svalid;
    if constexpr (kRows) valid = rows_below_count(s, c, p.row_count);
    float lown[2], best[2] = {-1.f, -1.f};
    int bidx[2] = {c.n0, c.n0};
#pragma unroll
    for (int h = 0; h < 2; ++h) lown[h] = ((valid >> h) & 1u) ? p.lse_own[c.sgrow[h]] : 0.f;
    constexpr int kSlices = (N + 31) / 32;
    float cmax[kSlices];
#pragma unroll
    for (int j = 0; j < kSlices; ++j) {
      const int col = 32 * j;
      cmax[j] = 0.f;
      if (col < c.ncols) {
        float v[16];
        frag_slice<N>(d, j, v);
        conf_slice(c, col, p.scale, lown, true, v, best, bidx);
        if constexpr (kRows) {
#pragma unroll
          for (int k = 0; k < 16; ++k)
            if (!((valid >> ((k >> 1) & 1)) & 1u)) v[k] = 0.f;
        }
        if (p.conf) conf_store(s, c, p.conf, col, v);
        float x[8];
#pragma unroll
        for (int k = 0; k < 8; ++k) {
          const float a = (valid & 1u) ? v[4 * (k >> 1) + (k & 1)] : 0.f;
          const float b = (valid & 2u) ? v[4 * (k >> 1) + 2 + (k & 1)] : 0.f;
          x[k] = fmaxf(a, b);
        }
        cmax[j] = col_reduce8(x, [](float a, float b) { return fmaxf(a, b); });
      }
    }
    conf_best_store(s, c, p.part_val, p.part_idx, best, bidx);
    const bool odd = (c.q & 1) != 0;
    const uint32_t xs = c.wstage_s + (odd ? 0 : kWarpStageBytes);
    if (odd) {
#pragma unroll
      for (int j = 0; j < kSlices; ++j) sts32f(xs + 4 * (32 * j + lane), cmax[j]);
    }
    pair_sync(c);
    if (!odd) {
      unsigned* cm = p.colmax + (long long)c.b * s.n_total + c.n0;
      const int lc = frag_lane_col();
#pragma unroll
      for (int j = 0; j < kSlices; ++j) {
        const int cl = 32 * j + lc;
        const float m = fmaxf(cmax[j], lds32f(xs + 4 * (32 * j + lane)));
        if (cl < c.ncols && m > 0.f) atomicMax(cm + cl, __float_as_uint(m));
      }
    }
    pair_sync(c);
  }
};

using EpiConfCol = EpiConfColT<false>;
using EpiConfColRows = EpiConfColT<true>;

template <int R>
__device__ __forceinline__ void wgmma_fence_acc(float (&d)[R]) {
#pragma unroll
  for (int i = 0; i < R; ++i) asm volatile("" : "+f"(d[i])::"memory");
}

template <int N, int KS>
__device__ __forceinline__ void mma_k_steps(float (&d)[N / 2], bool split, uint64_t a_hi, uint64_t a_lo,
                                            uint64_t b_hi, uint64_t b_lo) {
#pragma unroll
  for (int k = 0; k < KS; ++k) wgmma_m64nNk16<N>(d, a_hi + 2 * k, b_hi + 2 * k);
  if (split) {
#pragma unroll
    for (int k = 0; k < KS; ++k) wgmma_m64nNk16<N>(d, a_hi + 2 * k, b_lo + 2 * k);
#pragma unroll
    for (int k = 0; k < KS; ++k) wgmma_m64nNk16<N>(d, a_lo + 2 * k, b_hi + 2 * k);
  }
}

template <int A_MODE, class Epi, int BK>
__device__ __forceinline__ void gemm_body(const TensorMaps& maps, const GemmShape& s,
                                          const typename Epi::Params& ep) {
  static_assert(Epi::kGroups == 2, "each of the two MMA warpgroups is one epilogue group");
  static_assert(BK == 64 || BK == 32, "K chunk of one 128B- or 64B-swizzle row");
  constexpr int kABytes = gemm_a_bytes(BK);
  extern __shared__ uint8_t smem_raw[];
  uint8_t* smem = reinterpret_cast<uint8_t*>(
      (reinterpret_cast<uintptr_t>(smem_raw) + 1023) & ~static_cast<uintptr_t>(1023));
  const int planes = s.split ? 2 : 1;
  const bool nsc = s.pair == 2;
  constexpr int kParts = kBlockK / BK;
  const int slots = s.stages * kParts;
  const int b_bytes = s.mma_n * BK * 2;
  const int a_stage = kABytes * planes;
  const int b_stage = b_bytes * planes;
  const int ring = slots * (a_stage + b_stage);
  uint8_t* smem_a = smem;
  uint8_t* smem_b = smem + slots * a_stage;
  constexpr bool kAccTile = !EpiFromRegs<Epi>::value;
  uint8_t* smem_acc = s.acc_alias ? smem : smem + ring;
  float* epi_smem = reinterpret_cast<float*>(smem + ring + (kAccTile && !s.acc_alias ? gemm_acc_bytes(s.mma_n) : 0));
  uint64_t* bars = reinterpret_cast<uint64_t*>(reinterpret_cast<uint8_t*>(epi_smem) +
                                               epi_smem_bytes<Epi>());
  uint64_t* full = bars;
  uint64_t* empty = bars + kMaxStages;
  uint64_t* accfree = bars + 2 * kMaxStages;

  constexpr int kProducerWarp = 4 * Epi::kGroups;
  const int warp = threadIdx.x >> 5;
  const int lane = threadIdx.x & 31;
  const int csize = nsc ? 1 : s.cluster;
  const int prank = s.cluster > 1 ? (int)cluster_ctarank() : 0;
  const int crank = nsc ? 0 : prank;
  const int nrank = nsc ? prank : 0;
  const uint16_t cmask = (uint16_t)((1u << csize) - 1u);
  const int cluster_id = blockIdx.x / s.cluster;
  const int n_clusters = gridDim.x / s.cluster;
  const int tiles_per_batch = s.msup * s.n_tiles;
  const int total_tiles = s.batches * tiles_per_batch;

  if (warp == kProducerWarp && lane == 0) {
    tma_prefetch_desc(&maps.a[0]);
    tma_prefetch_desc(&maps.b);
  }
  if (warp == 0 && lane == 0) {
    for (int i = 0; i < slots; ++i) {
      mbar_init(&full[i], 1);
      mbar_init(&empty[i], 2 * csize);
    }
    mbar_init(accfree, 4 * Epi::kGroups * csize);
    if constexpr (EpiExtraSmem<Epi>::value > 0) {
      uint64_t* xbar = reinterpret_cast<uint64_t*>(reinterpret_cast<uint8_t*>(epi_smem) + epi_smem_bytes<Epi>() -
                                                   EpiExtraSmem<Epi>::value + 2 * 128 * 8);
      mbar_init(&xbar[0], Epi::kExchangeArrivals);
      mbar_init(&xbar[1], Epi::kExchangeArrivals);
    }
    fence_mbar_init();
  }
  if (s.cluster > 1) cluster_sync_all(); else __syncthreads();
  pdl_sync();

  if (warp >= kProducerWarp) {
    setmaxnreg_dec<kProducerRegs>();
    if (warp == kProducerWarp) {
      int stage = 0;
      uint32_t phase = 0;
      const bool skip_b = (s.debug_skip & 1) != 0, skip_a = (s.debug_skip & 2) != 0;
      const int a_tx = A_MODE == A_WIN ? s.tiles_x * s.tile_w * s.tile_h * (BK * 2) * planes : a_stage;
      const uint32_t tx_bytes = (skip_a ? 0 : a_tx) + (skip_b ? 0 : b_stage);
      int it = 0;
      for (int t = cluster_id; t < total_tiles; t += n_clusters, ++it) {
        if (s.acc_alias && it > 0) mbar_wait(accfree, (uint32_t)((it - 1) & 1));
        const int b = t / tiles_per_batch;
        const int r = t - b * tiles_per_batch;
        const int msi = r / s.n_tiles;
        const int n_tile = nsc ? nrank : r - msi * s.n_tiles;
        const int m_tile = msi * csize + crank;
        int ox0 = 0, oy0 = 0;
        if (A_MODE == A_CONV) {
          const int ty = m_tile / s.tiles_x;
          oy0 = ty * s.tile_h;
          ox0 = (m_tile - ty * s.tiles_x) * s.tile_w;
        }
        const int bb = s.b_batched ? b : 0;
        const int nrow0 = n_tile * s.block_n;
        int win_x[5] = {0, 0, 0, 0, 0}, win_y[5] = {0, 0, 0, 0, 0}, win_z[5] = {0, 0, 0, 0, 0};
        if constexpr (A_MODE == A_WIN) {
          const int cnt = s.rows / (s.tile_w * s.tile_h);
#pragma unroll
          for (int wi = 0; wi < 5; ++wi) {
            int m = m_tile * s.tiles_x + wi;
            m = m < cnt ? m : cnt - 1;
            win_z[wi] = m;
            if (ep.j_ids) {
              const int j = (int)ep.j_ids[m];
              const int cy = j / ep.wc;
              win_z[wi] = (int)ep.b_ids[m];
              win_x[wi] = ep.stride * (j - cy * ep.wc) + ep.org - s.conv_pad;
              win_y[wi] = ep.stride * cy + ep.org - s.conv_pad;
            }
          }
        }
        int cc = 0, ky = 0, kx = 0, kb_tap = 0;
        for (int chunk = 0; chunk < s.k_chunks; ++chunk) {
          const bool first = A_MODE == A_ROWS && chunk < s.k_chunks_a0;
          const int ka = A_MODE == A_ROWS ? (first ? chunk : chunk - s.k_chunks_a0) * kBlockK : cc * kBlockK;
          const int kb = A_MODE == A_ROWS ? chunk * kBlockK : kb_tap + ka;
#pragma unroll
          for (int part = 0; part < kParts; ++part) {
            const int kp = part * BK;
            mbar_wait(&empty[stage], phase ^ 1);
            uint8_t* sa = smem_a + stage * a_stage;
            uint8_t* sb = smem_b + stage * b_stage;
            {
              if constexpr (A_MODE == A_ROWS) {
                const CUtensorMap* am = first ? &maps.a[0] : &maps.a[1];
                const int lo = first ? s.a0_lo : s.a1_lo;
                const int ba = (first && s.a0_shared) ? 0 : b;
                if (elect_one()) {
                  mbar_expect_tx(&full[stage], tx_bytes);
                  if (!skip_a) {
                    tma_load_3d(am, &full[stage], sa, ka + kp, m_tile * kBlockM, ba);
                    if (s.split) tma_load_3d(am, &full[stage], sa + kABytes, ka + kp + lo, m_tile * kBlockM, ba);
                  }
                }
              } else if constexpr (A_MODE == A_WIN) {
                const int wbytes = s.tile_w * s.tile_h * (BK * 2);
#pragma unroll
                for (int wi = 0; wi < 5; ++wi) {
                  if (wi >= s.tiles_x) break;
                  const int bx = win_x[wi] + kx, by = win_y[wi] + ky, bz = win_z[wi];
                  if (elect_one()) {
                    if (wi == 0) mbar_expect_tx(&full[stage], tx_bytes);
                    if (!skip_a) {
                      tma_load_5d(&maps.a[0], &full[stage], sa + wi * wbytes, ka + kp, 0, bx, by, bz);
                      if (s.split)
                        tma_load_5d(&maps.a[0], &full[stage], sa + kABytes + wi * wbytes, ka + kp, 1, bx, by, bz);
                    }
                  }
                }
              } else {
                int dy = ky - s.conv_pad, dx = kx - s.conv_pad, mi = 0;
                if (s.conv_stride == 2) {
                  const int py = dy & 1, px = dx & 1;
                  dy = (dy - py) >> 1;
                  dx = (dx - px) >> 1;
                  mi = py * 2 + px;
                }
                const CUtensorMap* am = &maps.a[mi];
                if (elect_one()) {
                  mbar_expect_tx(&full[stage], tx_bytes);
                  if (!skip_a) {
                    tma_load_5d(am, &full[stage], sa, ka + kp, 0, ox0 + dx, oy0 + dy, b);
                    if (s.split) tma_load_5d(am, &full[stage], sa + kABytes, ka + kp, 1, ox0 + dx, oy0 + dy, b);
                  }
                }
              }
              if (!skip_b && elect_one()) {
                if (csize == 1) {
                  tma_load_3d(&maps.b, &full[stage], sb, kb + kp, nrow0, bb);
                  if (s.split) tma_load_3d(&maps.b, &full[stage], sb + b_bytes, s.b_lo + kb + kp, nrow0, bb);
                } else {
                  const int slice = s.mma_n / csize;
                  const int soff = crank * slice * (BK * 2);
                  const int nrow = nrow0 + crank * slice;
                  tma_load_3d_mc(&maps.b, &full[stage], sb + soff, kb + kp, nrow, bb, cmask);
                  if (s.split)
                    tma_load_3d_mc(&maps.b, &full[stage], sb + b_bytes + soff, s.b_lo + kb + kp, nrow, bb, cmask);
                }
              }
            }
            __syncwarp();
            if (++stage == slots) {
              stage = 0;
              phase ^= 1;
            }
          }
          if (A_MODE != A_ROWS && ++cc == s.conv_cchunks) {
            cc = 0;
            kb_tap += s.conv_c;
            if (++kx == s.conv_kw) {
              kx = 0;
              ++ky;
            }
          }
        }
      }
    }
  } else {
    setmaxnreg_inc<kMmaRegs>();
    const int g = warp >> 2;
    const int q = warp & 3;
    EpiCtx c;
    c.etid = q * 32 + lane;
    c.q = q;
    c.a_mode = A_MODE;
    c.group = g;
    c.col_first = 32 * g;
    c.col_step = 32 * Epi::kGroups;
    c.smem = epi_smem + g * (kEpiParamBytes / 8);
    c.wstage = reinterpret_cast<uint8_t*>(epi_smem) + kEpiParamBytes + warp * EpiWarpStage<Epi>::value;
    c.extra = reinterpret_cast<uint8_t*>(epi_smem) + epi_smem_bytes<Epi>() - EpiExtraSmem<Epi>::value;
    c.smem_s = smem_u32(c.smem);
    c.wstage_s = smem_u32(c.wstage);
    const uint64_t desc_tmpl = BK == 64 ? make_kmajor_sw128_desc(0) : make_kmajor_sw64_desc(0);
    const uint32_t sa0 = ((smem_u32(smem_a) >> 4) & 0x3FFF) + g * ((64 * BK * 2) >> 4);
    const uint32_t sb0 = (smem_u32(smem_b) >> 4) & 0x3FFF;
    const uint32_t a_step = (uint32_t)a_stage >> 4, b_step = (uint32_t)b_stage >> 4;
    const uint32_t a_lo_off = kABytes >> 4, b_lo_off = (uint32_t)b_bytes >> 4;
    const bool split = s.split != 0;
    const bool is_signal = q == 0 && lane == 0;
    const uint32_t pitch = (uint32_t)(s.mma_n + kAccPad);
    const uint32_t acc_w = smem_u32(smem_acc) >> 2;
    const uint32_t r0 = 64 * g + 16 * q + (lane >> 2), c0 = 2 * (lane & 3);
    auto release = [&](int st) {
      if (is_signal) {
        if (csize == 1) mbar_arrive(&empty[st]);
        else
          for (int r = 0; r < csize; ++r) mbar_arrive_cluster(&empty[st], (uint32_t)r);
      }
    };
    int stage = 0;
    uint32_t phase = 0;
    uint32_t sa = sa0, sb = sb0;
    const int tail_steps = (A_MODE != A_ROWS && (s.conv_c & 63)) ? (s.conv_c & 63) / 16 : 4;
    int it = 0;
    for (int t = cluster_id; t < total_tiles; t += n_clusters, ++it) {
      c.b = t / tiles_per_batch;
      const int r = t - c.b * tiles_per_batch;
      const int msi = r / s.n_tiles;
      c.n_tile = nsc ? nrank : r - msi * s.n_tiles;
      c.m_tile = msi * csize + crank;
      c.n0 = c.n_tile * s.block_n;
      const int rem = s.n_total - c.n0;
      c.ncols = rem < s.block_n ? rem : s.block_n;
      if constexpr (EpiNeedsNext<Epi>::value) {
        const int tn = t + n_clusters;
        c.next_b = -1;
        c.next_m_tile = 0;
        if (tn < total_tiles) {
          c.next_b = tn / tiles_per_batch;
          c.next_m_tile = ((tn - c.next_b * tiles_per_batch) / s.n_tiles) * csize + crank;
        }
      }
      c.it = it;
      c.svalid = 0;
      if constexpr (kAccTile) {
#pragma unroll
        for (int i = 0; i < 4; ++i) {
          int rdummy;
          if (epi_row_at(s, c, q * 32 + (lane >> 2) + 8 * i, c.sgrow[i], rdummy)) c.svalid |= 1u << i;
        }
      } else {
#pragma unroll
        for (int h = 0; h < 2; ++h) {
          int rdummy;
          if (epi_row_at(s, c, (int)r0 + 8 * h, c.sgrow[h], rdummy)) c.svalid |= 1u << h;
        }
      }
      c.acc = acc_w + (uint32_t)(q * 32 + lane) * pitch;
      Epi::prefetch(ep, s, c);

      auto mma_tile = [&](auto n_c, auto tail_c) {
        constexpr int N = decltype(n_c)::value;
        constexpr int TAIL = decltype(tail_c)::value;
        float d[N / 2];
#pragma unroll
        for (int i = 0; i < N / 2; ++i) d[i] = 0.f;
        wgmma_fence_acc(d);
        int prev = -1;
        static_assert(TAIL * 16 <= BK, "a tail chunk's channels lie in its first slot");
        auto chunk_step = [&](auto ks_c, auto& acc) {
          const uint64_t a_hi = desc_tmpl | sa, b_hi = desc_tmpl | sb;
          const uint64_t a_lo = desc_tmpl | (sa + a_lo_off), b_lo = desc_tmpl | (sb + b_lo_off);
          mbar_wait_hot(&full[stage], phase);
          wgmma_fence();
          mma_k_steps<N, decltype(ks_c)::value>(acc, split, a_hi, a_lo, b_hi, b_lo);
          wgmma_commit();
          wgmma_fence_acc(acc);
          if (prev >= 0) {
            wgmma_wait<1>();
            release(prev);
          }
          prev = stage;
          sa += a_step;
          sb += b_step;
          if (++stage == slots) {
            stage = 0;
            phase ^= 1;
            sa = sa0;
            sb = sb0;
          }
        };
        auto full_chunk = [&]() {
#pragma unroll
          for (int part = 0; part < kParts; ++part) chunk_step(std::integral_constant<int, BK / 16>{}, d);
        };
        auto tail_chunk = [&]() {
          chunk_step(std::integral_constant<int, TAIL>{}, d);
          if constexpr (kParts == 2) chunk_step(std::integral_constant<int, 0>{}, d);
        };
        if constexpr (TAIL == 0) {
          for (int chunk = 0; chunk < s.k_chunks; ++chunk) full_chunk();
        } else {
          const int taps = s.k_chunks / s.conv_cchunks;
          for (int tap = 0; tap < taps; ++tap) {
            for (int cc = 1; cc < s.conv_cchunks; ++cc) full_chunk();
            tail_chunk();
          }
        }
        wgmma_wait<0>();
        wgmma_fence_acc(d);
        if (prev >= 0) release(prev);

        if constexpr (!kAccTile) {
          if (!(s.debug_skip & 4)) Epi::template run_frag<N>(ep, s, c, d);
        } else {
          named_bar_sync(4, 256);
#pragma unroll
          for (int i = 0; i < N / 8; ++i) {
            const uint32_t col = 8 * i + c0;
            sts64f((acc_w + r0 * pitch + col) * 4, d[4 * i], d[4 * i + 1]);
            sts64f((acc_w + (r0 + 8) * pitch + col) * 4, d[4 * i + 2], d[4 * i + 3]);
          }
          named_bar_sync(4, 256);
        }
      };
      auto mma_width = [&](auto tail_c) {
        switch (s.mma_n) {
          case 64:
            if constexpr (EpiMinMmaN<Epi>::value <= 64) mma_tile(std::integral_constant<int, 64>{}, tail_c);
            break;
          case 128: mma_tile(std::integral_constant<int, 128>{}, tail_c); break;
          case 208: mma_tile(std::integral_constant<int, 208>{}, tail_c); break;
          default: mma_tile(std::integral_constant<int, 256>{}, tail_c); break;
        }
      };
      if constexpr (A_MODE == A_ROWS) {
        mma_width(std::integral_constant<int, 0>{});
      } else {
        switch (tail_steps) {
          case 1: mma_width(std::integral_constant<int, 1>{}); break;
          default: mma_width(std::integral_constant<int, 0>{}); break;
        }
      }

      if constexpr (kAccTile) {
        if (!(s.debug_skip & 4)) Epi::run(ep, s, c);
        if (s.acc_alias) {
          fence_proxy_async_smem();
          __syncwarp();
          if (lane == 0) {
            if (csize == 1) mbar_arrive(accfree);
            else
              for (int r2 = 0; r2 < csize; ++r2) mbar_arrive_cluster(accfree, (uint32_t)r2);
          }
        }
      }
    }
  }

  pdl_done();
  if (s.cluster > 1) cluster_sync_all(); else __syncthreads();
}

template <int A_MODE, class Epi, int BK = kBlockK>
__global__ void __launch_bounds__(gemm_threads(Epi::kGroups), 1)
gemm_kernel(const __grid_constant__ TensorMaps maps, const GemmShape s, const typename Epi::Params ep) {
  gemm_body<A_MODE, Epi, BK>(maps, s, ep);
}

template <int A_MODE, class Epi, int BK = kBlockK>
__global__ void __launch_bounds__(gemm_threads(Epi::kGroups), 1)
gemm_kernel_dyn(const __grid_constant__ TensorMaps maps, const GemmShape s_in,
                const typename Epi::Params ep, const int* rows_dev, int rows_mult) {
  GemmShape s = s_in;
  pdl_wait();
  const int r = *rows_dev * rows_mult;
  s.rows = r < s_in.rows ? r : s_in.rows;
  const int tile_rows = A_MODE == A_WIN ? s_in.tiles_x * s_in.tile_w * s_in.tile_h : kBlockM;
  s.m_tiles = (s.rows + tile_rows - 1) / tile_rows;
  s.msup = (s.m_tiles + s_in.cluster - 1) / s_in.cluster;
  gemm_body<A_MODE, Epi, BK>(maps, s, ep);
}

inline int gemm_stage_bytes(int mma_n, int split) {
  return (gemm_a_bytes(kBlockK) + mma_n * kBlockK * 2) * (split ? 2 : 1);
}
template <class Epi>
inline int gemm_smem_bytes(const GemmShape& s) {
  const bool acc_tile = !EpiFromRegs<Epi>::value && !s.acc_alias;
  return s.stages * gemm_stage_bytes(s.mma_n, s.split) + (acc_tile ? gemm_acc_bytes(s.mma_n) : 0) +
         epi_smem_bytes<Epi>() + (2 * kMaxStages + 2) * 8 + 16 + 1024;
}
constexpr int kSmemLimit = 227 * 1024;
template <class Epi>
inline bool gemm_pick_stages(GemmShape& s, int cap = 0) {
  const int avail = kSmemLimit - epi_smem_bytes<Epi>() - 2048;
  const int sb = gemm_stage_bytes(s.mma_n, s.split);
  const int max_st = kMaxStages * s.bk / kBlockK;
  const int ab = EpiFromRegs<Epi>::value ? 0 : gemm_acc_bytes(s.mma_n);
  int st = (avail - ab) / sb;
  s.acc_alias = ab > 0 && st < 2;
  if (s.acc_alias) st = avail / sb;
  if (st > max_st) st = max_st;
  if (st > s.k_chunks * 2 && s.k_chunks * 2 >= 2) st = s.k_chunks * 2;
  if (cap > 1 && st > cap) st = cap;
  if (st < 2) st = 2;
  if (s.acc_alias && st * sb < ab) st = (ab + sb - 1) / sb;
  s.stages = st;
  return st <= max_st && gemm_smem_bytes<Epi>(s) <= kSmemLimit;
}

}
```

Before: 478.1.

## Move conv_up epilogue to register fragments and drop the smem accumulator tile

The bilinear-upsample-add epilogue (EpiConvUp) now runs directly on the wgmma accumulator fragments. Before, it first staged the whole accumulator tile into shared memory and read it back. Each warp cp.async-copies a 20-pixel upsample window into a double-buffered warp stage and blends from there, replacing the per-lane global loads. With no epilogue still using the smem accumulator tile, that tile is removed along with the acc_alias mode and its barrier, and the freed shared memory goes to more pipeline stages. The window assumes each warp's fragment rows map to one output row of at most 20 source pixels, which ties correctness to the tile geometry.

```diff
diff --git a/onepose_plus_plus_b200/csrc/opp_gemm.cu b/onepose_plus_plus_b200/csrc/opp_gemm.cu
--- a/onepose_plus_plus_b200/csrc/opp_gemm.cu
+++ b/onepose_plus_plus_b200/csrc/opp_gemm.cu
@@ -102,8 +102,8 @@
   static int n_seen = 0;
   char key[128];
   snprintf(key, sizeof(key), "mode %d n %d block_n %d mma_n %d k %d conv_c %d stages %d alias %d cluster %d pair %d bk %d",
-           a_mode, s.n_total, s.block_n, s.mma_n, s.k_chunks * kBlockK, s.conv_c, s.stages, s.acc_alias,
-           s.cluster, s.pair, s.bk);
+           a_mode, s.n_total, s.block_n, s.mma_n, s.k_chunks * kBlockK, s.conv_c, s.stages, 0, s.cluster,
+           s.pair, s.bk);
   std::lock_guard<std::mutex> lock(mu);
   if (on == 2) {
     fprintf(stderr, "opp gemm tile: %s epi %s\n", key, epi);
@@ -179,9 +179,9 @@
   cudaError_t le = cudaLaunchKernelExC(&cfg, kern, kargs);
   if (le != cudaSuccess) {
     set_last_error("cudaLaunchKernelEx failed: %s (grid %d cluster %d pair %d smem %d stages %d "
-                   "acc_alias %d block_n %d m_tiles %d n_tiles %d batches %d)",
+                   "block_n %d m_tiles %d n_tiles %d batches %d)",
                    cudaGetErrorString(le), n_clusters * s.cluster, s.cluster, s.pair, smem, s.stages,
-                   s.acc_alias, s.block_n, s.m_tiles, s.n_tiles, s.batches);
+                   s.block_n, s.m_tiles, s.n_tiles, s.batches);
     return OPP_ERR_CUDA;
   }
   return OPP_OK;
diff --git a/onepose_plus_plus_b200/csrc/opp_gemm.cuh b/onepose_plus_plus_b200/csrc/opp_gemm.cuh
--- a/onepose_plus_plus_b200/csrc/opp_gemm.cuh
+++ b/onepose_plus_plus_b200/csrc/opp_gemm.cuh
@@ -49,7 +49,6 @@
   int cluster;
   int msup;
   int pair;
-  int acc_alias;
   int debug_skip;
   int split;
   int b_lo;
@@ -67,7 +66,6 @@
 };
 
 struct EpiCtx {
-  uint32_t acc;
   int b, m_tile, n_tile;
   int q;
   int a_mode;
@@ -78,19 +76,18 @@
   uint8_t* wstage;
   uint32_t smem_s, wstage_s;
   int group;
-  int col_first, col_step;
-  long long sgrow[4];
+  long long sgrow[2];
   unsigned svalid;
-  int next_b, next_m_tile;
   uint8_t* extra;
   int it;
 };
 
 __device__ __forceinline__ void epi_sync(const EpiCtx& c) { named_bar_sync(1 + c.group, 128); }
 
+constexpr int kWarpStageBytes = 2 * 16 * 80;
 template <class E, class = void>
 struct EpiWarpStage {
-  static constexpr int value = 32 * 80;
+  static constexpr int value = kWarpStageBytes;
 };
 template <class E>
 struct EpiWarpStage<E, std::void_t<decltype(E::kWarpStage)>> {
@@ -118,15 +115,6 @@
   static constexpr int value = E::kMinMmaN;
 };
 
-template <class E, class = void>
-struct EpiNeedsNext : std::false_type {};
-template <class E>
-struct EpiNeedsNext<E, std::void_t<decltype(E::kNeedsNext)>> : std::true_type {};
-
-template <class E, class = void>
-struct EpiFromRegs : std::false_type {};
-template <class E>
-struct EpiFromRegs<E, std::void_t<decltype(E::kFromRegs)>> : std::true_type {};
 
 __device__ __forceinline__ bool epi_row_at(const GemmShape& s, const EpiCtx& c, int rit,
                                            long long& grow, int& row) {
@@ -151,69 +139,10 @@
   return ok;
 }
 
-constexpr int kAccPad = 4;
-__host__ __device__ constexpr int gemm_acc_bytes(int mma_n) { return 128 * (mma_n + kAccPad) * 4; }
-
-__device__ __forceinline__ void acc_ld32(uint32_t waddr, float (&v)[32]) {
-#pragma unroll
-  for (int i = 0; i < 8; ++i) {
-    const uint4 u = lds128(waddr * 4 + 16 * i);
-    v[4 * i + 0] = __uint_as_float(u.x);
-    v[4 * i + 1] = __uint_as_float(u.y);
-    v[4 * i + 2] = __uint_as_float(u.z);
-    v[4 * i + 3] = __uint_as_float(u.w);
-  }
-}
-
-constexpr int kStageRowH = 80;
-constexpr int kWarpStageBytes = 32 * kStageRowH;
-
-__device__ __forceinline__ void staged_store_h32(const GemmShape& s, const EpiCtx& c, __half* out,
-                                                 long long ld, int lo_off, int gcol,
-                                                 const float* v, int nvalid) {
-  if (s.debug_skip & 8) return;
-  const int lane = threadIdx.x & 31;
-  const uint32_t st = c.wstage_s;
-#pragma unroll
-  for (int plane = 0; plane < 2; ++plane) {
-    if (plane == 1 && lo_off == 0) break;
-    const uint32_t mine = st + lane * kStageRowH;
-#pragma unroll
-    for (int g = 0; g < 4; ++g) {
-      uint4 u;
-      if (plane == 0) {
-        u.x = pack_half2(v[8 * g + 0], v[8 * g + 1]);
-        u.y = pack_half2(v[8 * g + 2], v[8 * g + 3]);
-        u.z = pack_half2(v[8 * g + 4], v[8 * g + 5]);
-        u.w = pack_half2(v[8 * g + 6], v[8 * g + 7]);
-      } else {
-        float l[8];
-#pragma unroll
-        for (int j = 0; j < 8; ++j)
-          l[j] = v[8 * g + j] - __half2float(__float2half_rn(v[8 * g + j]));
-        u.x = pack_half2(l[0], l[1]);
-        u.y = pack_half2(l[2], l[3]);
-        u.z = pack_half2(l[4], l[5]);
-        u.w = pack_half2(l[6], l[7]);
-      }
-      sts128(mine + g * 16, u);
-    }
-    __syncwarp();
-    const int seg = lane & 3;
-#pragma unroll
-    for (int i = 0; i < 4; ++i) {
-      const int rr = (lane >> 2) + 8 * i;
-      if (((c.svalid >> i) & 1u) && seg * 8 < nvalid)
-        *reinterpret_cast<uint4*>(out + c.sgrow[i] * ld + plane * lo_off + gcol + seg * 8) =
-            lds128(st + rr * kStageRowH + seg * 16);
-    }
-    __syncwarp();
-  }
-}
-
 
 constexpr int kFragRowH = 80;
 constexpr int kFragPlaneH = 16 * kFragRowH;
+static_assert(kWarpStageBytes == 2 * kFragPlaneH, "the default warp stage holds both planes of a slice");
 constexpr int kFragRowF = 160;
 
 __device__ __forceinline__ void sts32u(uint32_t addr, uint32_t v) {
@@ -254,10 +183,11 @@
 }
 
 __device__ __forceinline__ void frag_store_h(const GemmShape& s, const EpiCtx& c, __half* out, long long ld,
-                                             int lo_off, int gcol, const float (&v)[16], int nvalid) {
+                                             int lo_off, int gcol, const float (&v)[16], int nvalid,
+                                             uint32_t stage_off = 0) {
   if (s.debug_skip & 8) return;
   const int lane = threadIdx.x & 31, t = lane & 3, rq = lane >> 2;
-  const uint32_t st = c.wstage_s;
+  const uint32_t st = c.wstage_s + stage_off;
 #pragma unroll
   for (int ii = 0; ii < 4; ++ii)
 #pragma unroll
@@ -398,7 +328,6 @@
 struct EpiConv {
   static constexpr int kGroups = OPP_CONV_GROUPS;
   static constexpr const char* kName = "conv";
-  static constexpr bool kFromRegs = true;
   using Params = EpiConvParams;
   __device__ static void prefetch(const Params& p, const GemmShape& s, const EpiCtx& c) {
     if (!p.resid) return;
@@ -446,7 +375,6 @@
 struct EpiWin {
   static constexpr int kGroups = OPP_CONV_GROUPS;
   static constexpr const char* kName = "conv_win";
-  static constexpr bool kFromRegs = true;
   struct Params {
     __half* out;
     long long ld;
@@ -502,133 +430,127 @@
 struct EpiConvUp {
   static constexpr int kGroups = OPP_CONV_GROUPS;
   static constexpr const char* kName = "conv_up";
-  static constexpr bool kNeedsNext = true;
-  static constexpr int kWarpStage = 2 * 32 * 80;
+  static constexpr int kWinPx = 20;
+  static constexpr int kWinBytes = 2 * kWinPx * kFragRowH;
+  static constexpr int kWarpStage = 2 * kWinBytes;
+  static_assert(kWinBytes >= kWarpStageBytes, "a window buffer also serves frag_store_h");
   using Params = EpiConvParams;
 
   struct Geo {
     int ymin, xmin;
   };
-  __device__ static Geo window(const Params& p, const GemmShape& s, int m_tile, int q) {
+  __device__ static int tile_row(const EpiCtx& c) { return 4 * c.group + c.q; }
+  __device__ static Geo window(const Params& p, const GemmShape& s, int m_tile, int row) {
     const int ty = m_tile / s.tiles_x;
-    const int oy = min(ty * s.tile_h + (q * 32) / s.tile_w, s.out_h - 1);
+    const int oy = min(ty * s.tile_h + row, s.out_h - 1);
     const int ox = min((m_tile - ty * s.tiles_x) * s.tile_w, s.out_w - 1);
     return Geo{(int)(p.up_sy * (float)oy), (int)(p.up_sx * (float)ox)};
   }
-  __device__ static long long slot_pixel(const Params& p, int b, const Geo& g, int slot) {
-    const int sy_ = slot / 10, sx_ = slot - sy_ * 10;
+  __device__ static long long slot_pixel(const Params& p, int b, const Geo& g, int px) {
+    const int sy_ = px / 10, sx_ = px - sy_ * 10;
     return ((long long)b * p.up_h + min(g.ymin + sy_, p.up_h - 1)) * p.up_w + min(g.xmin + sx_, p.up_w - 1);
   }
+  __device__ static void copy_window(const Params& p, const GemmShape& s, const EpiCtx& c, int col, uint32_t buf) {
+    const int lane = threadIdx.x & 31, t = lane & 3, rq = lane >> 2;
+    const Geo g = window(p, s, c.m_tile, tile_row(c));
+    const bool ok = 8 * t < c.ncols - col;
+    const __half* upb = p.up + c.n0 + col + 8 * t;
+#pragma unroll
+    for (int i = 0; i < 5; ++i) {
+      const int sl = rq + 8 * i;
+      const int plane = sl >= kWinPx ? 1 : 0;
+      const bool in = ok && (plane == 0 || p.out_lo != 0);
+      const int px = (int)slot_pixel(p, c.b, g, sl - plane * kWinPx);
+      cp_async16_zfill(c.wstage_s + buf + sl * kFragRowH + 16 * t, in ? upb + (long long)px * p.ld + plane * p.out_lo : p.up,
+                       in ? 16 : 0);
+    }
+    cp_async_commit();
+  }
   __device__ static void prefetch(const Params& p, const GemmShape& s, const EpiCtx& c) {
-    if (c.next_b < 0) return;
+    if (s.debug_skip & 4) return;
+    copy_window(p, s, c, 0, 0);
+    if (32 < c.ncols) copy_window(p, s, c, 32, kWinBytes);
     const int lane = threadIdx.x & 31;
-    if (lane >= 30) return;
-    const Geo g = window(p, s, c.next_m_tile, c.q);
-    const char* px = reinterpret_cast<const char*>(p.up + slot_pixel(p, c.next_b, g, lane) * p.ld);
-    const int bytes = (p.out_lo ? 2 : 1) * s.n_total * 2;
-    for (int o = c.group * 128; o < bytes; o += 128 * kGroups) asm volatile("prefetch.global.L2 [%0];" ::"l"(px + o));
-  }
-  __device__ static void run(const Params& p, const GemmShape& s, const EpiCtx& c) {
-    epi_sync(c);
-    for (int i = c.etid; i < c.ncols; i += 128) sts32f(c.smem_s + 4 * i, p.bias[c.n0 + i]);
-    epi_sync(c);
-    const int lane = threadIdx.x & 31;
-    const int seg = lane & 3;
-    const Geo g = window(p, s, c.m_tile, c.q);
-    float w00, w01, w10, w11;
-    uint32_t a00, a01, a10, a11;
-    {
-      const int rit = c.q * 32 + lane;
-      const int ty = c.m_tile / s.tiles_x;
-      const int ly = rit / s.tile_w;
-      const int oy = min(ty * s.tile_h + ly, s.out_h - 1);
-      const int ox = min((c.m_tile - ty * s.tiles_x) * s.tile_w + (rit - ly * s.tile_w), s.out_w - 1);
-      const float fy = p.up_sy * (float)oy, fx = p.up_sx * (float)ox;
-      const int y0 = (int)fy, x0 = (int)fx;
-      const int y1 = y0 + (y0 < p.up_h - 1 ? 1 : 0), x1 = x0 + (x0 < p.up_w - 1 ? 1 : 0);
-      const float wy = fy - (float)y0, wx = fx - (float)x0;
-      w00 = (1.f - wy) * (1.f - wx);
-      w01 = (1.f - wy) * wx;
-      w10 = wy * (1.f - wx);
-      w11 = wy * wx;
-      a00 = c.wstage_s + ((y0 - g.ymin) * 10 + (x0 - g.xmin)) * kStageRowH;
-      a01 = c.wstage_s + ((y0 - g.ymin) * 10 + (x1 - g.xmin)) * kStageRowH;
-      a10 = c.wstage_s + ((y1 - g.ymin) * 10 + (x0 - g.xmin)) * kStageRowH;
-      a11 = c.wstage_s + ((y1 - g.ymin) * 10 + (x1 - g.xmin)) * kStageRowH;
-    }
-    int spix[4];
-#pragma unroll
-    for (int i = 0; i < 4; ++i) spix[i] = (int)slot_pixel(p, c.b, g, min((lane >> 2) + 8 * i, 29));
-    const __half* upb = p.up + seg * 8 + c.n0;
+    if (64 >= c.ncols || lane >= kWinPx) return;
+    const Geo g = window(p, s, c.m_tile, tile_row(c));
+    const char* px = reinterpret_cast<const char*>(p.up + slot_pixel(p, c.b, g, lane) * p.ld + c.n0);
+#pragma unroll
+    for (int plane = 0; plane < 2; ++plane) {
+      if (plane == 1 && p.out_lo == 0) break;
+      const char* row = px + 2 * plane * p.out_lo;
+      for (int o = 128; o < 2 * c.ncols; o += 128) asm volatile("prefetch.global.L2 [%0];" ::"l"(row + o));
+      asm volatile("prefetch.global.L2 [%0];" ::"l"(row + 2 * c.ncols - 2));
+    }
+  }
+  template <int N>
+  __device__ __forceinline__ static void run_frag(const Params& p, const GemmShape& s, const EpiCtx& c, float (&d)[N / 2]) {
+    const int t = threadIdx.x & 3, rq = (threadIdx.x & 31) >> 2;
     const bool two = p.out_lo != 0;
-    uint4 nb[8];
-    auto issue = [&](int col) {
-      const bool ok = seg * 8 < c.ncols - col;
-#pragma unroll
-      for (int i = 0; i < 4; ++i) {
-        const __half* px = upb + (long long)spix[i] * p.ld + col;
-        nb[i] = ok ? *reinterpret_cast<const uint4*>(px) : make_uint4(0, 0, 0, 0);
-        nb[4 + i] = (ok && two) ? *reinterpret_cast<const uint4*>(px + p.out_lo) : make_uint4(0, 0, 0, 0);
-      }
-    };
-    constexpr uint32_t kLo = 32 * kStageRowH;
-    auto stage = [&]() {
-#pragma unroll
-      for (int i = 0; i < 4; ++i) {
-        const uint32_t a = c.wstage_s + ((lane >> 2) + 8 * i) * kStageRowH + seg * 16;
-        sts128(a, nb[i]);
-        if (two) sts128(a + kLo, nb[4 + i]);
-      }
+    const Geo g = window(p, s, c.m_tile, tile_row(c));
+    const int ty = c.m_tile / s.tiles_x;
+    const int oy = min(ty * s.tile_h + tile_row(c), s.out_h - 1);
+    const float fy = p.up_sy * (float)oy;
+    const int y0 = (int)fy;
+    const int y1 = y0 + (y0 < p.up_h - 1 ? 1 : 0);
+    const float wy = fy - (float)y0;
+    float w00[2], w01[2], w10[2], w11[2];
+    uint32_t o00[2], o01[2], o10[2], o11[2];
+#pragma unroll
+    for (int h = 0; h < 2; ++h) {
+      const int ox = min((c.m_tile - ty * s.tiles_x) * s.tile_w + rq + 8 * h, s.out_w - 1);
+      const float fx = p.up_sx * (float)ox;
+      const int x0 = (int)fx;
+      const int x1 = x0 + (x0 < p.up_w - 1 ? 1 : 0);
+      const float wx = fx - (float)x0;
+      w00[h] = (1.f - wy) * (1.f - wx);
+      w01[h] = (1.f - wy) * wx;
+      w10[h] = wy * (1.f - wx);
+      w11[h] = wy * wx;
+      o00[h] = ((y0 - g.ymin) * 10 + (x0 - g.xmin)) * kFragRowH + 4 * t;
+      o01[h] = ((y0 - g.ymin) * 10 + (x1 - g.xmin)) * kFragRowH + 4 * t;
+      o10[h] = ((y1 - g.ymin) * 10 + (x0 - g.xmin)) * kFragRowH + 4 * t;
+      o11[h] = ((y1 - g.ymin) * 10 + (x1 - g.xmin)) * kFragRowH + 4 * t;
+    }
+    auto blend = [&](uint32_t buf, float (&v)[16]) {
+#pragma unroll
+      for (int ii = 0; ii < 4; ++ii)
+#pragma unroll
+        for (int h = 0; h < 2; ++h)
+#pragma unroll
+          for (int plane = 0; plane < 2; ++plane) {
+            if (plane == 1 && !two) break;
+            const uint32_t b = buf + plane * (kWinPx * kFragRowH) + 16 * ii;
+            const uint32_t u00 = lds32u(b + o00[h]), u01 = lds32u(b + o01[h]);
+            const uint32_t u10 = lds32u(b + o10[h]), u11 = lds32u(b + o11[h]);
+            const float2 fa = __half22float2(*reinterpret_cast<const __half2*>(&u00));
+            const float2 fb = __half22float2(*reinterpret_cast<const __half2*>(&u01));
+            const float2 fc = __half22float2(*reinterpret_cast<const __half2*>(&u10));
+            const float2 fd = __half22float2(*reinterpret_cast<const __half2*>(&u11));
+            v[4 * ii + 2 * h] += (w00[h] * fa.x + w01[h] * fb.x) + (w10[h] * fc.x + w11[h] * fd.x);
+            v[4 * ii + 2 * h + 1] += (w00[h] * fa.y + w01[h] * fb.y) + (w10[h] * fc.y + w11[h] * fd.y);
+          }
       __syncwarp();
     };
-    auto blend = [&](float* v) {
-#pragma unroll
-      for (int q4 = 0; q4 < 4; ++q4) {
-#pragma unroll
-        for (int plane = 0; plane < 2; ++plane) {
-          if (plane == 1 && !two) break;
-          const uint32_t o = plane * kLo + q4 * 16;
-          const uint4 q00 = lds128(a00 + o), q01 = lds128(a01 + o);
-          const uint4 q10 = lds128(a10 + o), q11 = lds128(a11 + o);
-          const __half2* h00 = reinterpret_cast<const __half2*>(&q00);
-          const __half2* h01 = reinterpret_cast<const __half2*>(&q01);
-          const __half2* h10 = reinterpret_cast<const __half2*>(&q10);
-          const __half2* h11 = reinterpret_cast<const __half2*>(&q11);
-#pragma unroll
-          for (int j = 0; j < 4; ++j) {
-            const float2 fa = __half22float2(h00[j]), fb = __half22float2(h01[j]);
-            const float2 fc = __half22float2(h10[j]), fd = __half22float2(h11[j]);
-            v[8 * q4 + 2 * j] += (w00 * fa.x + w01 * fb.x) + (w10 * fc.x + w11 * fd.x);
-            v[8 * q4 + 2 * j + 1] += (w00 * fa.y + w01 * fb.y) + (w10 * fc.y + w11 * fd.y);
-          }
-        }
-      }
-      __syncwarp();
-    };
-    if (c.col_first < c.ncols) issue(c.col_first);
-    for (int col = c.col_first; col < c.ncols; col += c.col_step) {
-      float v[32];
-      acc_ld32(c.acc + col, v);
-#pragma unroll
-      for (int q4 = 0; q4 < 8; ++q4) {
-        const uint4 bq = lds128(c.smem_s + 4 * ((col + 4 * q4) & 255));
-        v[4 * q4 + 0] += __uint_as_float(bq.x);
-        v[4 * q4 + 1] += __uint_as_float(bq.y);
-        v[4 * q4 + 2] += __uint_as_float(bq.z);
-        v[4 * q4 + 3] += __uint_as_float(bq.w);
-      }
-      stage();
-      const int ncol = col + c.col_step;
-      if (ncol < c.ncols) issue(ncol);
-      blend(v);
-      if (p.act == 1) {
-#pragma unroll
-        for (int j = 0; j < 32; ++j) v[j] = fmaxf(v[j], 0.f);
-      } else if (p.act == 2) {
-#pragma unroll
-        for (int j = 0; j < 32; ++j) v[j] = v[j] > 0.f ? v[j] : v[j] * p.slope;
-      }
-      staged_store_h32(s, c, p.out, p.ld, p.out_lo, c.n0 + col, v, c.ncols - col);
+    epi_stage_cols(s, c, p.bias);
+#pragma unroll
+    for (int j = 0; j < (N + 31) / 32; ++j) {
+      const int col = 32 * j;
+      if (col < c.ncols) {
+        const uint32_t cur = (j & 1) ? kWinBytes : 0;
+        float v[16];
+        frag_slice<N>(d, j, v);
+        frag_add_cols(c.smem_s, col, v);
+        if (col + 32 < c.ncols) {
+          if (j > 0) copy_window(p, s, c, col + 32, kWinBytes - cur);
+          cp_async_wait<1>();
+        } else {
+          cp_async_wait<0>();
+        }
+        __syncwarp();
+        blend(c.wstage_s + cur, v);
+        frag_act(p.act, p.slope, v);
+        frag_store_h(s, c, p.out, p.ld, p.out_lo, c.n0 + col, v, c.ncols - col, cur);
+      }
     }
   }
 };
@@ -697,7 +619,6 @@
 struct EpiStoreF16 {
   static constexpr int kGroups = 2;
   static constexpr const char* kName = "store_f16";
-  static constexpr bool kFromRegs = true;
   struct Params {
     __half* out;
     long long ld;
@@ -742,7 +663,6 @@
 struct EpiQ {
   static constexpr int kGroups = 2;
   static constexpr const char* kName = "q";
-  static constexpr bool kFromRegs = true;
   struct Params {
     __half* out;
     long long ld;
@@ -797,7 +717,6 @@
 struct EpiLN {
   static constexpr int kGroups = 2;
   static constexpr const char* kName = "ln";
-  static constexpr bool kFromRegs = true;
   static constexpr int kExtraSmem = 2 * 128 * 8 + 64;
   static constexpr int kExchangeArrivals = 64;
   struct Params {
@@ -912,7 +831,6 @@
 struct EpiLse {
   static constexpr int kGroups = 2;
   static constexpr const char* kName = "lse";
-  static constexpr bool kFromRegs = true;
   struct Params {
     float* part_m;
     float* part_s;
@@ -1001,7 +919,6 @@
 struct EpiConf {
   static constexpr int kGroups = 2;
   static constexpr const char* kName = "conf";
-  static constexpr bool kFromRegs = true;
   struct Params {
     const float* lse_own;
     const float* lse_other;
@@ -1056,7 +973,6 @@
   static_assert(!(kMask && kRows), "query_image_mask and per-batch row counts are not combined");
   static constexpr int kGroups = 2;
   static constexpr const char* kName = kRows ? "lse_col_rows" : "lse_col";
-  static constexpr bool kFromRegs = true;
   static constexpr int kMinMmaN = 128;
   using Params = std::conditional_t<kRows, EpiLseColRowsParams, EpiLseColParams>;
   __device__ static void prefetch(const Params&, const GemmShape&, const EpiCtx&) {}
@@ -1174,7 +1090,6 @@
 struct EpiConfColT {
   static constexpr int kGroups = 2;
   static constexpr const char* kName = kRows ? "conf_col_rows" : "conf_col";
-  static constexpr bool kFromRegs = true;
   static constexpr int kMinMmaN = 128;
   using Params = std::conditional_t<kRows, EpiConfColRowsParams, EpiConfColParams>;
   __device__ static void prefetch(const Params&, const GemmShape&, const EpiCtx&) {}
@@ -1277,14 +1192,11 @@
   const int ring = slots * (a_stage + b_stage);
   uint8_t* smem_a = smem;
   uint8_t* smem_b = smem + slots * a_stage;
-  constexpr bool kAccTile = !EpiFromRegs<Epi>::value;
-  uint8_t* smem_acc = s.acc_alias ? smem : smem + ring;
-  float* epi_smem = reinterpret_cast<float*>(smem + ring + (kAccTile && !s.acc_alias ? gemm_acc_bytes(s.mma_n) : 0));
+  float* epi_smem = reinterpret_cast<float*>(smem + ring);
   uint64_t* bars = reinterpret_cast<uint64_t*>(reinterpret_cast<uint8_t*>(epi_smem) +
                                                epi_smem_bytes<Epi>());
   uint64_t* full = bars;
   uint64_t* empty = bars + kMaxStages;
-  uint64_t* accfree = bars + 2 * kMaxStages;
 
   constexpr int kProducerWarp = 4 * Epi::kGroups;
   const int warp = threadIdx.x >> 5;
@@ -1308,7 +1220,6 @@
       mbar_init(&full[i], 1);
       mbar_init(&empty[i], 2 * csize);
     }
-    mbar_init(accfree, 4 * Epi::kGroups * csize);
     if constexpr (EpiExtraSmem<Epi>::value > 0) {
       uint64_t* xbar = reinterpret_cast<uint64_t*>(reinterpret_cast<uint8_t*>(epi_smem) + epi_smem_bytes<Epi>() -
                                                    EpiExtraSmem<Epi>::value + 2 * 128 * 8);
@@ -1330,7 +1241,6 @@
       const uint32_t tx_bytes = (skip_a ? 0 : a_tx) + (skip_b ? 0 : b_stage);
       int it = 0;
       for (int t = cluster_id; t < total_tiles; t += n_clusters, ++it) {
-        if (s.acc_alias && it > 0) mbar_wait(accfree, (uint32_t)((it - 1) & 1));
         const int b = t / tiles_per_batch;
         const int r = t - b * tiles_per_batch;
         const int msi = r / s.n_tiles;
@@ -1456,8 +1366,6 @@
     c.q = q;
     c.a_mode = A_MODE;
     c.group = g;
-    c.col_first = 32 * g;
-    c.col_step = 32 * Epi::kGroups;
     c.smem = epi_smem + g * (kEpiParamBytes / 8);
     c.wstage = reinterpret_cast<uint8_t*>(epi_smem) + kEpiParamBytes + warp * EpiWarpStage<Epi>::value;
     c.extra = reinterpret_cast<uint8_t*>(epi_smem) + epi_smem_bytes<Epi>() - EpiExtraSmem<Epi>::value;
@@ -1470,9 +1378,7 @@
     const uint32_t a_lo_off = kABytes >> 4, b_lo_off = (uint32_t)b_bytes >> 4;
     const bool split = s.split != 0;
     const bool is_signal = q == 0 && lane == 0;
-    const uint32_t pitch = (uint32_t)(s.mma_n + kAccPad);
-    const uint32_t acc_w = smem_u32(smem_acc) >> 2;
-    const uint32_t r0 = 64 * g + 16 * q + (lane >> 2), c0 = 2 * (lane & 3);
+    const uint32_t r0 = 64 * g + 16 * q + (lane >> 2);
     auto release = [&](int st) {
       if (is_signal) {
         if (csize == 1) mbar_arrive(&empty[st]);
@@ -1494,31 +1400,13 @@
       c.n0 = c.n_tile * s.block_n;
       const int rem = s.n_total - c.n0;
       c.ncols = rem < s.block_n ? rem : s.block_n;
-      if constexpr (EpiNeedsNext<Epi>::value) {
-        const int tn = t + n_clusters;
-        c.next_b = -1;
-        c.next_m_tile = 0;
-        if (tn < total_tiles) {
-          c.next_b = tn / tiles_per_batch;
-          c.next_m_tile = ((tn - c.next_b * tiles_per_batch) / s.n_tiles) * csize + crank;
-        }
-      }
       c.it = it;
       c.svalid = 0;
-      if constexpr (kAccTile) {
-#pragma unroll
-        for (int i = 0; i < 4; ++i) {
-          int rdummy;
-          if (epi_row_at(s, c, q * 32 + (lane >> 2) + 8 * i, c.sgrow[i], rdummy)) c.svalid |= 1u << i;
-        }
-      } else {
-#pragma unroll
-        for (int h = 0; h < 2; ++h) {
-          int rdummy;
-          if (epi_row_at(s, c, (int)r0 + 8 * h, c.sgrow[h], rdummy)) c.svalid |= 1u << h;
-        }
-      }
-      c.acc = acc_w + (uint32_t)(q * 32 + lane) * pitch;
+#pragma unroll
+      for (int h = 0; h < 2; ++h) {
+        int rdummy;
+        if (epi_row_at(s, c, (int)r0 + 8 * h, c.sgrow[h], rdummy)) c.svalid |= 1u << h;
+      }
       Epi::prefetch(ep, s, c);
 
       auto mma_tile = [&](auto n_c, auto tail_c) {
@@ -1573,18 +1461,7 @@
         wgmma_fence_acc(d);
         if (prev >= 0) release(prev);
 
-        if constexpr (!kAccTile) {
-          if (!(s.debug_skip & 4)) Epi::template run_frag<N>(ep, s, c, d);
-        } else {
-          named_bar_sync(4, 256);
-#pragma unroll
-          for (int i = 0; i < N / 8; ++i) {
-            const uint32_t col = 8 * i + c0;
-            sts64f((acc_w + r0 * pitch + col) * 4, d[4 * i], d[4 * i + 1]);
-            sts64f((acc_w + (r0 + 8) * pitch + col) * 4, d[4 * i + 2], d[4 * i + 3]);
-          }
-          named_bar_sync(4, 256);
-        }
+        if (!(s.debug_skip & 4)) Epi::template run_frag<N>(ep, s, c, d);
       };
       auto mma_width = [&](auto tail_c) {
         switch (s.mma_n) {
@@ -1602,19 +1479,6 @@
         switch (tail_steps) {
           case 1: mma_width(std::integral_constant<int, 1>{}); break;
           default: mma_width(std::integral_constant<int, 0>{}); break;
-        }
-      }
-
-      if constexpr (kAccTile) {
-        if (!(s.debug_skip & 4)) Epi::run(ep, s, c);
-        if (s.acc_alias) {
-          fence_proxy_async_smem();
-          __syncwarp();
-          if (lane == 0) {
-            if (csize == 1) mbar_arrive(accfree);
-            else
-              for (int r2 = 0; r2 < csize; ++r2) mbar_arrive_cluster(accfree, (uint32_t)r2);
-          }
         }
       }
     }
@@ -1649,9 +1513,8 @@
 }
 template <class Epi>
 inline int gemm_smem_bytes(const GemmShape& s) {
-  const bool acc_tile = !EpiFromRegs<Epi>::value && !s.acc_alias;
-  return s.stages * gemm_stage_bytes(s.mma_n, s.split) + (acc_tile ? gemm_acc_bytes(s.mma_n) : 0) +
-         epi_smem_bytes<Epi>() + (2 * kMaxStages + 2) * 8 + 16 + 1024;
+  return s.stages * gemm_stage_bytes(s.mma_n, s.split) + epi_smem_bytes<Epi>() + (2 * kMaxStages + 2) * 8 + 16 +
+         1024;
 }
 constexpr int kSmemLimit = 227 * 1024;
 template <class Epi>
@@ -1659,15 +1522,11 @@
   const int avail = kSmemLimit - epi_smem_bytes<Epi>() - 2048;
   const int sb = gemm_stage_bytes(s.mma_n, s.split);
   const int max_st = kMaxStages * s.bk / kBlockK;
-  const int ab = EpiFromRegs<Epi>::value ? 0 : gemm_acc_bytes(s.mma_n);
-  int st = (avail - ab) / sb;
-  s.acc_alias = ab > 0 && st < 2;
-  if (s.acc_alias) st = avail / sb;
+  int st = avail / sb;
   if (st > max_st) st = max_st;
   if (st > s.k_chunks * 2 && s.k_chunks * 2 >= 2) st = s.k_chunks * 2;
   if (cap > 1 && st > cap) st = cap;
   if (st < 2) st = 2;
-  if (s.acc_alias && st * sb < ab) st = (ab + sb - 1) / sb;
   s.stages = st;
   return st <= max_st && gemm_smem_bytes<Epi>(s) <= kSmemLimit;
 }
```

Measured after the change: 478.3 (median of 6 runs). Within noise of the previous version (+0.0%).
